# cheneeheng/2s-AGCN

Hardware: AMD Instinct MI355X
Metric: skeleton-clips/sec fwd+bwd, NTU (N,3,300,25,2) (higher is better)
Workload: dtype f32; 1 GPU; AGCN joint-stream NTU-xview shape, full training step (fwd, CE, bwd, grad all-reduce, clip 1.0, SGD nesterov); per_gpu_batch=64, global_batch=64, input=(N,3,300,25,2), parallelism=dp1, bn=per-replica

## Files before the change

2s-agcn_amd/csrc/bn.hip:

```cpp
#include "agcn_common.h"

namespace {

constexpr int RG = 64;

__global__ void __launch_bounds__(256)
colsum_stage1_kernel(const float* __restrict__ X, int nslots, int W, int per_group, double* __restrict__ partial) {
  __shared__ double red[4][64];
  const int col = blockIdx.x * 64 + (threadIdx.x & 63), sub = threadIdx.x >> 6;
  const int g = blockIdx.y;
  const int s_end = min(nslots, (g + 1) * per_group);
  double acc = 0.0;
  if (col < W)
    for (int s = g * per_group + sub; s < s_end; s += 4) acc += (double)X[(long)s * W + col];
  red[sub][threadIdx.x & 63] = acc;
  __syncthreads();
  if (sub == 0 && col < W)
    partial[(long)g * W + col] = red[0][threadIdx.x] + red[1][threadIdx.x] + red[2][threadIdx.x] + red[3][threadIdx.x];
}

__global__ void colsum_stage2_kernel(const double* __restrict__ partial, int W, float* __restrict__ out) {
  const int col = blockIdx.x * blockDim.x + threadIdx.x;
  if (col >= W) return;
  double s = 0.0;
  for (int g = 0; g < RG; ++g) s += partial[(long)g * W + col];
  out[col] = (float)s;
}

__global__ void bn_stats_finalize_kernel(const double* __restrict__ partial, int C, double count,
                                         const float* __restrict__ gamma, const float* __restrict__ beta,
                                         float* __restrict__ rmean, float* __restrict__ rvar, float momentum,
                                         float eps, float* __restrict__ mean_out, float* __restrict__ invstd_out,
                                         float* __restrict__ scale_out, float* __restrict__ shift_out) {
  const int c = blockIdx.x * blockDim.x + threadIdx.x;
  if (c >= C) return;
  double s = 0.0, ss = 0.0;
  for (int g = 0; g < RG; ++g) {
    s += partial[((long)g * 2 + 0) * C + c];
    ss += partial[((long)g * 2 + 1) * C + c];
  }
  const double mean = s / count;
  double var = ss / count - mean * mean;
  if (var < 0.0) var = 0.0;
  const float invstd = (float)(1.0 / sqrt(var + (double)eps));
  mean_out[c] = (float)mean;
  invstd_out[c] = invstd;
  const float sc = gamma[c] * invstd;
  scale_out[c] = sc;
  shift_out[c] = beta[c] - (float)mean * sc;
  if (rmean) {
    const double unb = count > 1.0 ? var * count / (count - 1.0) : var;
    rmean[c] = (1.f - momentum) * rmean[c] + momentum * (float)mean;
    rvar[c] = (1.f - momentum) * rvar[c] + momentum * (float)unb;
  }
}

__global__ void bn_eval_coeff_kernel(const float* __restrict__ gamma, const float* __restrict__ beta,
                                     const float* __restrict__ rmean, const float* __restrict__ rvar, float eps, int C,
                                     float* __restrict__ scale_out, float* __restrict__ shift_out) {
  const int c = blockIdx.x * blockDim.x + threadIdx.x;
  if (c >= C) return;
  const float sc = gamma[c] / sqrtf(rvar[c] + eps);
  scale_out[c] = sc;
  shift_out[c] = beta[c] - rmean[c] * sc;
}

template <int RES, bool RELU>
__global__ void __launch_bounds__(256)
bn_act_fwd_kernel(const float4* __restrict__ y1, const float* __restrict__ scale1, const float* __restrict__ shift1,
                  const float4* __restrict__ r, const float* __restrict__ scale2, const float* __restrict__ shift2,
                  float4* __restrict__ out, unsigned* __restrict__ bits, unsigned total4, unsigned P, unsigned C,
                  unsigned* __restrict__ amax) {
  unsigned tmax = 0;
  for (unsigned i0 = blockIdx.x * blockDim.x; i0 < total4; i0 += gridDim.x * blockDim.x) {
    const unsigned i = i0 + threadIdx.x;
    const bool valid = i < total4;
    const unsigned ic = valid ? i : 0u;
    const unsigned e0 = ic * 4u;
    const unsigned row = e0 / P;
    const unsigned rem = e0 - row * P;
    const unsigned c0 = row % C;
    const unsigned c1 = (c0 + 1 == C) ? 0u : c0 + 1;
    const float4 a = y1[ic];
    float4 b = make_float4(0.f, 0.f, 0.f, 0.f);
    if (RES != 0) b = r[ic];
    float av[4] = {a.x, a.y, a.z, a.w};
    float bv[4] = {b.x, b.y, b.z, b.w};
    float ov[4];
#pragma unroll
    for (int k = 0; k < 4; ++k) {
      const unsigned c = (rem + k < P) ? c0 : c1;
      float v = scale1[c] * av[k] + shift1[c];
      if (RES == 1) v += bv[k];
      if (RES == 2) v += scale2[c] * bv[k] + shift2[c];
      ov[k] = RELU ? fmaxf(v, 0.f) : v;
    }
    if (valid) out[i] = make_float4(ov[0], ov[1], ov[2], ov[3]);
    if (amax && valid) {
#pragma unroll
      for (int k = 0; k < 4; ++k) tmax = max(tmax, __float_as_uint(ov[k]) & 0x7fffffffu);
    }
    if (bits) {
      unsigned nib = valid ? ((ov[0] > 0.f) | ((ov[1] > 0.f) << 1) | ((ov[2] > 0.f) << 2) | ((ov[3] > 0.f) << 3)) : 0u;
      unsigned w = nib << (4u * (threadIdx.x & 7u));
      w |= __shfl_xor(w, 1);
      w |= __shfl_xor(w, 2);
      w |= __shfl_xor(w, 4);
      if ((threadIdx.x & 7u) == 0u && valid) bits[e0 >> 5] = w;
    }
  }
  if (amax) {
#pragma unroll
    for (int k = 32; k >= 1; k >>= 1) tmax = max(tmax, (unsigned)__shfl_xor((int)tmax, k));
    __shared__ unsigned wmax[4];
    if ((threadIdx.x & 63u) == 0u) wmax[threadIdx.x >> 6] = tmax;
    __syncthreads();
    if (threadIdx.x == 0) {
      const unsigned m = max(max(wmax[0], wmax[1]), max(wmax[2], wmax[3]));
      if (m) atomicMax(amax, m);
    }
  }
}

template <bool HAS2>
__global__ void __launch_bounds__(256)
bn_bwd_reduce_kernel(const float* __restrict__ dout, const float* __restrict__ mask, int mask_bits,
                     const float* __restrict__ y1, const float* __restrict__ y2, float* __restrict__ part, int P) {
  __shared__ float red[3][4];
  const long row = blockIdx.x;
  const float* d = dout + row * P;
  const float* mk = (mask && !mask_bits) ? mask + row * P : nullptr;
  const unsigned* mb = (mask && mask_bits) ? reinterpret_cast<const unsigned*>(mask) : nullptr;
  const long e_row = row * P;
  const float* a = y1 + row * P;
  const float* b = HAS2 ? y2 + row * P : nullptr;
  float s0 = 0.f, s1 = 0.f, s2 = 0.f;
  typedef float4 float4_u __attribute__((aligned(4)));
  const int P4 = P >> 2;
  for (int q4 = threadIdx.x; q4 < P4; q4 += 256) {
    const float4 d4 = reinterpret_cast<const float4_u*>(d)[q4];
    const float4 a4 = reinterpret_cast<const float4_u*>(a)[q4];
    float dv[4] = {d4.x, d4.y, d4.z, d4.w};
    const float av[4] = {a4.x, a4.y, a4.z, a4.w};
    if (mk) {
      const float4 m4 = reinterpret_cast<const float4_u*>(mk)[q4];
      const float mv[4] = {m4.x, m4.y, m4.z, m4.w};
#pragma unroll
      for (int k = 0; k < 4; ++k) dv[k] = (mv[k] > 0.f) ? dv[k] : 0.f;
    }
    if (mb) {
      const long e = e_row + 4L * q4;
      const int sh = (int)(e & 31);
      unsigned nib = mb[e >> 5] >> sh;
      if (sh > 28) nib |= mb[(e >> 5) + 1] << (32 - sh);
#pragma unroll
      for (int k = 0; k < 4; ++k) dv[k] = ((nib >> k) & 1u) ? dv[k] : 0.f;
    }
    float bv[4] = {0.f, 0.f, 0.f, 0.f};
    if (HAS2) {
      const float4 b4 = reinterpret_cast<const float4_u*>(b)[q4];
      bv[0] = b4.x; bv[1] = b4.y; bv[2] = b4.z; bv[3] = b4.w;
    }
#pragma unroll
    for (int k = 0; k < 4; ++k) {
      s0 += dv[k];
      s1 += dv[k] * av[k];
      if (HAS2) s2 += dv[k] * bv[k];
    }
  }
  for (int q = 4 * P4 + threadIdx.x; q < P; q += 256) {
    float dz = d[q];
    if (mk) dz = (mk[q] > 0.f) ? dz : 0.f;
    if (mb) {
      const long e = e_row + q;
      dz = ((mb[e >> 5] >> (e & 31)) & 1u) ? dz : 0.f;
    }
    s0 += dz;
    s1 += dz * a[q];
    if (HAS2) s2 += dz * b[q];
  }
  s0 = half_sum(s0); s1 = half_sum(s1); s2 = half_sum(s2);
  s0 += __shfl_xor(s0, 32); s1 += __shfl_xor(s1, 32); s2 += __shfl_xor(s2, 32);
  const int wave = threadIdx.x >> 6;
  if ((threadIdx.x & 63) == 0) { red[0][wave] = s0; red[1][wave] = s1; red[2][wave] = s2; }
  __syncthreads();
  if (threadIdx.x < 3) {
    const int k = threadIdx.x;
    part[row * 3 + k] = red[k][0] + red[k][1] + red[k][2] + red[k][3];
  }
}

__global__ void bn_bwd_finalize_kernel(const float* __restrict__ part, int N, int C, double count, float pscale,
                                       const float* __restrict__ gamma1, const float* __restrict__ mean1,
                                       const float* __restrict__ invstd1, const float* __restrict__ gamma2,
                                       const float* __restrict__ mean2, const float* __restrict__ invstd2,
                                       float* __restrict__ coef, float* __restrict__ dgamma1,
                                       float* __restrict__ dbeta1, float* __restrict__ dgamma2,
                                       float* __restrict__ dbeta2) {
  const int c = blockIdx.x * blockDim.x + threadIdx.x;
  if (c >= C) return;
  double s0 = 0.0, s1 = 0.0, s2 = 0.0;
#pragma unroll 8
  for (int n = 0; n < N; ++n) {
    const float* p = part + ((long)n * C + c) * 3;
    s0 += (double)p[0]; s1 += (double)p[1]; s2 += (double)p[2];
  }
  {
    const double is = invstd1[c], mu = mean1[c], g = gamma1[c];
    const double sxh = is * (s1 - mu * s0);
    const double k = g * is;
    coef[0 * C + c] = (float)k;
    coef[1 * C + c] = (float)(-k * is * sxh / count);
    coef[2 * C + c] = (float)(-k * s0 / count + k * is * mu * sxh / count);
    dgamma1[c] = (float)sxh * pscale;
    dbeta1[c] = (float)s0 * pscale;
  }
  if (gamma2) {
    const double is = invstd2[c], mu = mean2[c], g = gamma2[c];
    const double sxh = is * (s2 - mu * s0);
    const double k = g * is;
    coef[3 * C + c] = (float)k;
    coef[4 * C + c] = (float)(-k * is * sxh / count);
    coef[5 * C + c] = (float)(-k * s0 / count + k * is * mu * sxh / count);
    dgamma2[c] = (float)sxh * pscale;
    dbeta2[c] = (float)s0 * pscale;
  }
}

template <bool HAS2>
__global__ void __launch_bounds__(256)
bn_bwd_apply_kernel(const float4* __restrict__ dout, const float4* __restrict__ mask, int mask_bits,
                    const float4* __restrict__ y1,
                    const float4* __restrict__ y2, const float* __restrict__ coef, float4* __restrict__ dy1,
                    float4* __restrict__ dy2, unsigned total4, unsigned P, unsigned C, unsigned* __restrict__ amax1) {
  unsigned tmax = 0;
  for (unsigned i = blockIdx.x * blockDim.x + threadIdx.x; i < total4; i += gridDim.x * blockDim.x) {
    const unsigned e0 = i * 4u;
    const unsigned row = e0 / P;
    const unsigned rem = e0 - row * P;
    const unsigned c0 = row % C;
    const unsigned c1 = (c0 + 1 == C) ? 0u : c0 + 1;
    const float4 d4 = dout[i];
    const float4 a4 = y1[i];
    float dv[4] = {d4.x, d4.y, d4.z, d4.w};
    float av[4] = {a4.x, a4.y, a4.z, a4.w};
    if (mask && !mask_bits) {
      const float4 m4 = mask[i];
      const float mv[4] = {m4.x, m4.y, m4.z, m4.w};
#pragma unroll
      for (int k = 0; k < 4; ++k) dv[k] = (mv[k] > 0.f) ? dv[k] : 0.f;
    } else if (mask) {
      const unsigned nib = reinterpret_cast<const unsigned*>(mask)[e0 >> 5] >> (e0 & 31u);
#pragma unroll
      for (int k = 0; k < 4; ++k) dv[k] = ((nib >> k) & 1u) ? dv[k] : 0.f;
    }
    float bv[4] = {0.f, 0.f, 0.f, 0.f};
    if (HAS2) {
      const float4 b4 = y2[i];
      bv[0] = b4.x; bv[1] = b4.y; bv[2] = b4.z; bv[3] = b4.w;
    }
    float o1[4], o2[4];
#pragma unroll
    for (int k = 0; k < 4; ++k) {
      const unsigned c = (rem + k < P) ? c0 : c1;
      o1[k] = coef[0 * C + c] * dv[k] + coef[1 * C + c] * av[k] + coef[2 * C + c];
      if (HAS2) o2[k] = coef[3 * C + c] * dv[k] + coef[4 * C + c] * bv[k] + coef[5 * C + c];
    }
    dy1[i] = make_float4(o1[0], o1[1], o1[2], o1[3]);
    if (HAS2) dy2[i] = make_float4(o2[0], o2[1], o2[2], o2[3]);
    if (amax1) {
#pragma unroll
      for (int k = 0; k < 4; ++k) tmax = max(tmax, __float_as_uint(o1[k]) & 0x7fffffffu);
    }
  }
  if (amax1) {
#pragma unroll
    for (int k = 32; k >= 1; k >>= 1) tmax = max(tmax, (unsigned)__shfl_xor((int)tmax, k));
    __shared__ unsigned wmax[4];
    if ((threadIdx.x & 63u) == 0u) wmax[threadIdx.x >> 6] = tmax;
    __syncthreads();
    if (threadIdx.x == 0) {
      const unsigned m = max(max(wmax[0], wmax[1]), max(wmax[2], wmax[3]));
      if (m) atomicMax(amax1, m);
    }
  }
}

inline unsigned ew_grid(unsigned total4) {
  unsigned g = (total4 + 255u) / 256u;
  return g > 4096u ? 4096u : (g ? g : 1u);
}

}

extern "C" {

size_t agcn_colsum_scratch_bytes(int W) { return sizeof(double) * (size_t)RG * (size_t)W; }

int agcn_colsum(const float* X, int nslots, int W, void* scratch, float* out, void* stream) {
  if (!X || !scratch || !out || nslots <= 0 || W <= 0) return AGCN_ERR_ARG;
  hipStream_t s = (hipStream_t)stream;
  const int per_group = (nslots + RG - 1) / RG;
  hipLaunchKernelGGL(colsum_stage1_kernel, dim3((W + 63) / 64, RG), dim3(256), 0, s, X, nslots, W, per_group,
                     (double*)scratch);
  int rc = agcn_check_launch();
  if (rc) return rc;
  hipLaunchKernelGGL(colsum_stage2_kernel, dim3((W + 255) / 256), dim3(256), 0, s, (const double*)scratch, W, out);
  return agcn_check_launch();
}

int agcn_bn_stats_finalize(const float* part, int nslots, int C, double count, const float* gamma, const float* beta,
                           float* running_mean, float* running_var, float momentum, float eps, void* scratch,
                           float* mean, float* invstd, float* scale, float* shift, void* stream) {
  if (!part || !gamma || !beta || !scratch || !mean || !invstd || !scale || !shift || C <= 0 || nslots <= 0)
    return AGCN_ERR_ARG;
  hipStream_t s = (hipStream_t)stream;
  const int W = 2 * C;
  const int per_group = (nslots + RG - 1) / RG;
  hipLaunchKernelGGL(colsum_stage1_kernel, dim3((W + 63) / 64, RG), dim3(256), 0, s, part, nslots, W, per_group,
                     (double*)scratch);
  int rc = agcn_check_launch();
  if (rc) return rc;
  hipLaunchKernelGGL(bn_stats_finalize_kernel, dim3((C + 63) / 64), dim3(64), 0, s, (const double*)scratch, C, count,
                     gamma, beta, running_mean, running_var, momentum, eps, mean, invstd, scale, shift);
  return agcn_check_launch();
}

int agcn_bn_eval_coeff(const float* gamma, const float* beta, const float* running_mean, const float* running_var,
                       float eps, int C, float* scale, float* shift, void* stream) {
  if (!gamma || !beta || !running_mean || !running_var || !scale || !shift || C <= 0) return AGCN_ERR_ARG;
  hipLaunchKernelGGL(bn_eval_coeff_kernel, dim3((C + 63) / 64), dim3(64), 0, (hipStream_t)stream, gamma, beta,
                     running_mean, running_var, eps, C, scale, shift);
  return agcn_check_launch();
}

int agcn_bn_act_fwd(const float* y1, const float* scale1, const float* shift1, const float* r, const float* scale2,
                    const float* shift2, float* out, unsigned* sign_bits, int N, int C, int P, int res_mode, int relu,
                    void* stream) {
  return agcn_bn_act_fwd_ex(y1, scale1, shift1, r, scale2, shift2, out, sign_bits, nullptr, N, C, P, res_mode, relu, stream);
}

int agcn_bn_act_fwd_ex(const float* y1, const float* scale1, const float* shift1, const float* r, const float* scale2,
                       const float* shift2, float* out, unsigned* sign_bits, float* absmax_out, int N, int C, int P,
                       int res_mode, int relu, void* stream) {
  if (!y1 || !scale1 || !shift1 || !out || N <= 0 || C <= 0 || P <= 0) return AGCN_ERR_ARG;
  if (absmax_out && hipMemsetAsync(absmax_out, 0, 4, (hipStream_t)stream) != hipSuccess) return AGCN_ERR_ARG;
  const long total = (long)N * C * P;
  if (total % 4 != 0 || total > 0xffffffffL) return AGCN_ERR_UNSUPPORTED;
  if (res_mode != 0 && !r) return AGCN_ERR_ARG;
  if (res_mode == 2 && (!scale2 || !shift2)) return AGCN_ERR_ARG;
  const unsigned t4 = (unsigned)(total / 4);
  hipStream_t s = (hipStream_t)stream;
  const dim3 g(ew_grid(t4)), b(256);
#define LAUNCH_ACT(R, A)                                                                                       \
  hipLaunchKernelGGL((bn_act_fwd_kernel<R, A>), g, b, 0, s, (const float4*)y1, scale1, shift1, (const float4*)r, \
                     scale2, shift2, (float4*)out, sign_bits, t4, (unsigned)P, (unsigned)C, (unsigned*)absmax_out)
  if (relu) {
    if (res_mode == 0) LAUNCH_ACT(0, true); else if (res_mode == 1) LAUNCH_ACT(1, true); else LAUNCH_ACT(2, true);
  } else {
    if (res_mode == 0) LAUNCH_ACT(0, false); else if (res_mode == 1) LAUNCH_ACT(1, false); else LAUNCH_ACT(2, false);
  }
#undef LAUNCH_ACT
  return agcn_check_launch();
}

int agcn_bn_bwd_reduce(const float* dout, const void* mask, int mask_bits, const float* y1, const float* y2, float* part,
                       int N, int C, int P, void* stream) {
  if (!dout || !y1 || !part || N <= 0 || C <= 0 || P <= 0) return AGCN_ERR_ARG;
  hipStream_t s = (hipStream_t)stream;
  if (y2) hipLaunchKernelGGL(bn_bwd_reduce_kernel<true>, dim3(N * C), dim3(256), 0, s, dout, (const float*)mask,
                             mask_bits, y1, y2, part, P);
  else hipLaunchKernelGGL(bn_bwd_reduce_kernel<false>, dim3(N * C), dim3(256), 0, s, dout, (const float*)mask,
                          mask_bits, y1, y2, part, P);
  return agcn_check_launch();
}

int agcn_bn_bwd_apply(const float* part, int nrows, double count, float param_grad_scale, const float* dout,
                      const void* mask, int mask_bits, const float* y1, const float* gamma1, const float* mean1, const float* invstd1,
                      const float* y2, const float* gamma2, const float* mean2, const float* invstd2, float* coef,
                      float* dy1, float* dgamma1, float* dbeta1, float* dy2, float* dgamma2, float* dbeta2, int N, int C,
                      int P, void* stream) {
  return agcn_bn_bwd_apply_ex(part, nrows, count, param_grad_scale, dout, mask, mask_bits, y1, gamma1, mean1, invstd1, y2,
                              gamma2, mean2, invstd2, coef, dy1, dgamma1, dbeta1, dy2, dgamma2, dbeta2, nullptr, N, C, P,
                              stream);
}

int agcn_bn_bwd_apply_ex(const float* part, int nrows, double count, float param_grad_scale, const float* dout,
                         const void* mask, int mask_bits, const float* y1, const float* gamma1, const float* mean1,
                         const float* invstd1, const float* y2, const float* gamma2, const float* mean2,
                         const float* invstd2, float* coef, float* dy1, float* dgamma1, float* dbeta1, float* dy2,
                         float* dgamma2, float* dbeta2, float* absmax1_out, int N, int C, int P, void* stream) {
  if (absmax1_out && hipMemsetAsync(absmax1_out, 0, 4, (hipStream_t)stream) != hipSuccess) return AGCN_ERR_ARG;
  if (!part || !dout || !y1 || !gamma1 || !mean1 || !invstd1 || !coef || !dy1 || !dgamma1 || !dbeta1 || nrows <= 0)
    return AGCN_ERR_ARG;
  if (y2 && (!gamma2 || !mean2 || !invstd2 || !dy2 || !dgamma2 || !dbeta2)) return AGCN_ERR_ARG;
  const long total = (long)N * C * P;
  if (total % 4 != 0 || total > 0xffffffffL) return AGCN_ERR_UNSUPPORTED;
  hipStream_t s = (hipStream_t)stream;
  hipLaunchKernelGGL(bn_bwd_finalize_kernel, dim3((C + 63) / 64), dim3(64), 0, s, part, nrows, C, count,
                     param_grad_scale, gamma1, mean1, invstd1, y2 ? gamma2 : nullptr, mean2, invstd2, coef, dgamma1,
                     dbeta1, dgamma2, dbeta2);
  int rc = agcn_check_launch();
  if (rc) return rc;
  const unsigned t4 = (unsigned)(total / 4);
  const dim3 g(ew_grid(t4)), b(256);
  if (y2)
    hipLaunchKernelGGL(bn_bwd_apply_kernel<true>, g, b, 0, s, (const float4*)dout, (const float4*)mask, mask_bits,
                       (const float4*)y1, (const float4*)y2, (const float*)coef, (float4*)dy1, (float4*)dy2, t4,
                       (unsigned)P, (unsigned)C, (unsigned*)absmax1_out);
  else
    hipLaunchKernelGGL(bn_bwd_apply_kernel<false>, g, b, 0, s, (const float4*)dout, (const float4*)mask, mask_bits,
                       (const float4*)y1, (const float4*)y2, (const float*)coef, (float4*)dy1, (float4*)dy2, t4,
                       (unsigned)P, (unsigned)C, (unsigned*)absmax1_out);
  return agcn_check_launch();
}

int agcn_bn_bwd(const float* dout, const void* mask, int mask_bits, const float* y1, const float* gamma1,
                const float* mean1, const float* invstd1, const float* y2, const float* gamma2, const float* mean2,
                const float* invstd2, float* part, float* coef, float* dy1, float* dgamma1, float* dbeta1, float* dy2,
                float* dgamma2, float* dbeta2, int N, int C, int P, void* stream) {
  int rc = agcn_bn_bwd_reduce(dout, mask, mask_bits, y1, y2, part, N, C, P, stream);
  if (rc) return rc;
  return agcn_bn_bwd_apply(part, N, (double)N * (double)P, 1.0f, dout, mask, mask_bits, y1, gamma1, mean1, invstd1, y2, gamma2,
                           mean2, invstd2, coef, dy1, dgamma1, dbeta1, dy2, dgamma2, dbeta2, N, C, P, stream);
}

const char* agcn_arch(void) { return "gfx950"; }
int agcn_version(void) { return 100; }

}
```

2s-agcn_amd/lib.py:

```python
import ctypes
import os
import re

import torch

_HERE = os.path.dirname(os.path.abspath(__file__))
LIB_PATH = os.path.join(_HERE, "libagcn_hip.so")
HEADER_PATH = os.path.join(os.path.dirname(_HERE), "include", "agcn_hip.h")

_RETURNS = {"int": ctypes.c_int, "size_t": ctypes.c_size_t, "const char*": ctypes.c_char_p}
_SCALARS = {"int": ctypes.c_int, "long": ctypes.c_long, "size_t": ctypes.c_size_t, "float": ctypes.c_float,
            "double": ctypes.c_double}
_FP32, _FP64, _INT32 = ("fp32", (torch.float32,)), ("float64", (torch.float64,)), ("int32", (torch.int32,))
_BITS32, _ANY = ("int32", (torch.int32, torch.uint32)), ("", None)
_POINTERS = {"float*": _FP32, "const float*": _FP32, "double*": _FP64, "const double*": _FP64,
             "int*": _INT32, "const int*": _INT32, "unsigned*": _BITS32, "const unsigned*": _BITS32,
             "const long long*": ("int64", (torch.int64,)), "const unsigned char*": ("uint8", (torch.uint8,)),
             "void*": _ANY, "const void*": _ANY}
_TYPE_WORDS = {"const", "void", "char", "int", "long", "unsigned", "signed", "short", "float", "double", "size_t"}


def _c_type(tokens):
    return " ".join(tokens).replace(" *", "*")


def parse_header(text):
    text = re.sub(r"/\*.*?\*/|//[^\n]*", " ", text, flags=re.S)
    codes = {m.group(1): int(m.group(2))
             for m in re.finditer(r"^[ \t]*#[ \t]*define[ \t]+(AGCN_\w+)[ \t]+\(?(-?\d+)\)?[ \t]*$", text, flags=re.M)}
    text = re.sub(r"^[ \t]*#.*$", " ", text, flags=re.M)
    text = re.sub(r'extern\s+"C"\s*\{', " ", text)
    decls = {}
    for chunk in text.split(";"):
        decl = " ".join(chunk.split())
        if decl in ("", "}"):
            continue
        m = re.fullmatch(r"([\w\s*]+?)\b(\w+) ?\(([^()]*)\)", decl)
        if m is None:
            raise RuntimeError(f"agcn_amd: cannot read the declaration `{decl}` of the C ABI header")
        ret, name = _c_type(m.group(1).replace("*", " * ").split()), m.group(2)
        if ret not in _RETURNS:
            raise RuntimeError(f"agcn_amd: return type `{ret}` outside the binding's set in `{decl}`")
        params = []
        for p in ([] if m.group(3).strip() in ("", "void") else m.group(3).split(",")):
            tokens = p.replace("*", " * ").split()
            if len(tokens) < 2 or tokens[-1] == "*" or tokens[-1] in _TYPE_WORDS:
                raise RuntimeError(f"agcn_amd: parameter `{p.strip()}` has no name in `{decl}`")
            ctype = _c_type(tokens[:-1])
            if ctype not in _SCALARS and ctype not in _POINTERS:
                raise RuntimeError(f"agcn_amd: parameter type `{ctype}` outside the binding's set in `{decl}`")
            params.append((ctype, tokens[-1]))
        decls[name] = (ret, params)
    return decls, codes


def _read_header():
    try:
        with open(HEADER_PATH) as f:
            return f.read()
    except OSError as e:
        raise RuntimeError(f"agcn_amd: the C ABI header {HEADER_PATH} is missing ({e}); the binding is derived from "
                           f"it") from e


def _pointer_converter(ctype, where):
    kind, dtypes = _POINTERS[ctype]
    want = f"{where}: expected a contiguous {kind + ' ' if kind else ''}GPU tensor"

    def convert(t):
        if t is None or type(t) is int:
            return t
        if not (t.is_cuda and t.is_contiguous() and (dtypes is None or t.dtype in dtypes)):
            raise RuntimeError(f"agcn_amd: {want}, got {t.dtype} {tuple(t.shape)} on {t.device} "
                               f"contiguous={t.is_contiguous()}")
        return t.data_ptr()
    return convert


def _host_ints_converter(where):
    def convert(values):
        if values is None:
            return None
        if torch.is_tensor(values):
            if values.is_cuda or values.dtype.is_floating_point or values.dtype == torch.bool:
                raise RuntimeError(f"agcn_amd: {where}: expected a host sequence of ints, got {values.dtype} on "
                                   f"{values.device}")
            values = values.tolist()
        values = list(values)
        if any(isinstance(v, bool) or int(v) != v for v in values):
            raise RuntimeError(f"agcn_amd: {where}: expected a host sequence of ints, got {values!r}")
        return (ctypes.c_int * len(values))(*[int(v) for v in values])
    return convert


def _converter(ctype, pname, name):
    if pname.startswith("host_"):
        assert ctype == "const int*", f"{name}({pname}): host arrays are `const int*`"
        return _host_ints_converter(f"{name}({pname})")
    return _pointer_converter(ctype, f"{name}({pname})")


DECLARATIONS, _CODES = parse_header(_read_header())
ERR_ARG, ERR_WORKSPACE, ERR_UNSUPPORTED = (_CODES[k] for k in ("AGCN_ERR_ARG", "AGCN_ERR_WORKSPACE",
                                                                "AGCN_ERR_UNSUPPORTED"))
SIGNATURES = {name: (_RETURNS[ret], [_SCALARS.get(t, ctypes.c_void_p) for t, _ in params])
              for name, (ret, params) in DECLARATIONS.items()}
_CONVERTERS = {}
for _name, (_ret, _params) in DECLARATIONS.items():
    if any(t in _POINTERS for t, _ in _params):
        assert _ret == "int" and _params[-1] == ("void*", "stream"), f"{_name}: not `int {_name}(..., void* stream)`"
        _CONVERTERS[_name] = tuple(_converter(t, p, _name) if t in _POINTERS else None for t, p in _params[:-1])

_lib = None


def load():
    global _lib
    if _lib is not None:
        return _lib
    if not os.path.exists(LIB_PATH):
        raise RuntimeError(
            f"agcn_amd: HIP extension {LIB_PATH} not found -- run `python -c 'import __graft_entry__ as g; "
            f"g.build()'` (hipcc --offload-arch=gfx950).  There is no CPU fallback for the hot path.")
    lib = ctypes.CDLL(LIB_PATH)
    for name, (res, args) in SIGNATURES.items():
        fn = getattr(lib, name)
        fn.restype = res
        fn.argtypes = args
    _lib = lib
    return lib


ptr = _pointer_converter("const float*", "ptr")
ptr.__doc__ = "Device pointer of a tensor (None -> NULL).  The tensor must be contiguous fp32 on a GPU."
ptr_bits = _pointer_converter("const int*", "ptr_bits")
ptr_bits.__doc__ = "Device pointer of an int32 sign-bit-mask tensor (None -> NULL)."


def stream():
    return torch.cuda.current_stream().cuda_stream


def check(rc, what):
    if rc != 0:
        raise RuntimeError(f"agcn_amd: {what} failed with code {rc}")


def status(name, *args):
    convert = _CONVERTERS.get(name)
    if convert is None:
        raise RuntimeError(f"agcn_amd: {name} is not a stream entry point of include/agcn_hip.h")
    if len(args) != len(convert):
        raise RuntimeError(f"agcn_amd: {name} takes {len(convert)} arguments in front of the stream, got {len(args)}")
    return getattr(_lib or load(), name)(*[a if c is None else c(a) for c, a in zip(convert, args)], stream())


def call(name, *args):
    check(status(name, *args), name)
```

2s-agcn_amd/model/agcn.py:

```python
import math

import numpy as np
import torch
import torch.nn as nn

from .. import ops


def import_class(name):
    import importlib
    module_name, _, cls = name.rpartition('.')
    return getattr(importlib.import_module(module_name), cls)


def conv_branch_init(conv, branches):
    out_c, in_c, k = conv.weight.size(0), conv.weight.size(1), conv.weight.size(2)
    nn.init.normal_(conv.weight, 0, math.sqrt(2.0 / (out_c * in_c * k * branches)))
    nn.init.constant_(conv.bias, 0)


def conv_init(conv):
    nn.init.kaiming_normal_(conv.weight, mode='fan_out')
    nn.init.constant_(conv.bias, 0)


def bn_init(bn, scale):
    nn.init.constant_(bn.weight, scale)
    nn.init.constant_(bn.bias, 0)


def _require_gpu(x, who):
    if not x.is_cuda:
        raise RuntimeError(f"agcn_amd.{who}: input is on {x.device}; the hot path exists only as gfx950 HIP kernels "
                           f"(no CPU fallback). Move the model and data to a GPU.")
    if x.dtype != torch.float32:
        raise RuntimeError(f"agcn_amd.{who}: expected float32 input, got {x.dtype}")


def _bn_args(bn):
    return bn.weight, bn.bias, bn.running_mean, bn.running_var


def _bn_tick(bn, training):
    if training and bn.num_batches_tracked is not None:
        bn.num_batches_tracked.add_(1)


def _conv_bn_args(conv, bn):
    return (conv.weight, conv.bias) + _bn_args(bn)


def gcn_params(g, ab, A, PA, alpha=None):
    return dict(conv_d=[(c.weight, c.bias) for c in g.conv_d],
                ab=None if ab is None else [(a.weight, a.bias, b.weight, b.bias) for a, b in zip(ab.conv_a, ab.conv_b)],
                A=A, PA=PA, alpha=alpha, gbn=_bn_args(g.bn),
                down=_conv_bn_args(*g.down) if isinstance(g.down, nn.Sequential) else None)


def unit_params(unit, p, attn=None):
    t, r = unit.tcn1, unit.residual
    p.update(tw=t.conv.weight, tb=t.conv.bias, tbn=_bn_args(t.bn), res_mode=unit.res_mode,
             res=_conv_bn_args(r.conv, r.bn) if unit.res_mode == 2 else None, stride=unit.stride, pad=t.pad, attn=attn)
    return p


def data_bn_forward(bn, x):
    N, C, T, V, M = x.size()
    if ops.data_bn_supported(bn):
        y = ops.DataBNFunction.apply(x, bn.weight, bn.bias, bn.running_mean, bn.running_var, bn.training,
                                     ops.sync_of(bn))
        _bn_tick(bn, bn.training)
        return y
    x = x.permute(0, 4, 3, 1, 2).contiguous().view(N, M * V * C, T)
    x = bn(x)
    return x.view(N, M, V, C, T).permute(0, 1, 3, 4, 2).contiguous().view(N * M, C, T, V)


class unit_tcn(nn.Module):
    def __init__(self, in_channels, out_channels, kernel_size=9, stride=1):
        super().__init__()
        if not 1 <= kernel_size <= 9:
            raise NotImplementedError(f"agcn_amd.unit_tcn: kernel_size {kernel_size} is outside 1..9, the temporal "
                                      f"kernel sizes the HIP convolution kernels are built for")
        pad = int((kernel_size - 1) / 2)
        self.conv = nn.Conv2d(in_channels, out_channels, kernel_size=(kernel_size, 1), padding=(pad, 0),
                              stride=(stride, 1))
        self.bn = nn.BatchNorm2d(out_channels)
        self.relu = nn.ReLU()
        self.stride, self.pad = stride, pad
        conv_init(self.conv)
        bn_init(self.bn, 1)

    def forward(self, x):
        _require_gpu(x, 'unit_tcn')
        y = ops.UnitTCNFunction.apply(x, self.conv.weight, self.conv.bias, *_bn_args(self.bn), self.stride,
                                      self.training, ops.sync_of(self.bn), self.pad)
        _bn_tick(self.bn, self.training)
        return y


class unit_gcn(nn.Module):
    def __init__(self, in_channels, out_channels, A, coff_embedding=4, num_subset=3):
        super().__init__()
        if num_subset != 3:
            raise ValueError("agcn_amd.unit_gcn: num_subset must be 3")
        inter_channels = out_channels // coff_embedding
        self.inter_c = inter_channels
        self.in_channels, self.out_channels = in_channels, out_channels
        A = np.asarray(A, dtype=np.float32)
        self.PA = nn.Parameter(torch.full(A.shape, 1e-6, dtype=torch.float32))
        self.register_buffer('A', torch.from_numpy(A.copy()), persistent=False)
        self.num_subset = num_subset
        self.conv_a = nn.ModuleList()
        self.conv_b = nn.ModuleList()
        self.conv_d = nn.ModuleList()
        for _ in range(num_subset):
            self.conv_a.append(nn.Conv2d(in_channels, inter_channels, 1))
            self.conv_b.append(nn.Conv2d(in_channels, inter_channels, 1))
            self.conv_d.append(nn.Conv2d(in_channels, out_channels, 1))
        if in_channels != out_channels:
            self.down = nn.Sequential(nn.Conv2d(in_channels, out_channels, 1), nn.BatchNorm2d(out_channels))
        else:
            self.down = lambda x: x
        self.bn = nn.BatchNorm2d(out_channels)
        self.soft = nn.Softmax(-2)
        self.relu = nn.ReLU()
        for m in self.modules():
            if isinstance(m, nn.Conv2d):
                conv_init(m)
            elif isinstance(m, nn.BatchNorm2d):
                bn_init(m, 1)
        bn_init(self.bn, 1e-6)
        for i in range(num_subset):
            conv_branch_init(self.conv_d[i], num_subset)

    def params(self):
        return gcn_params(self, self, self.A, self.PA)

    def tick(self):
        _bn_tick(self.bn, self.training)
        if isinstance(self.down, nn.Sequential):
            _bn_tick(self.down[1], self.training)

    def forward(self, x):
        _require_gpu(x, 'unit_gcn')
        y = ops.UnitGCNFunction.apply(x, *ops.pack_gcn(self.params()), self.training, None, ops.sync_of(self.bn))
        self.tick()
        return y


class TCN_GCN_unit(nn.Module):
    def __init__(self, in_channels, out_channels, A, stride=1, residual=True):
        super().__init__()
        self.gcn1 = unit_gcn(in_channels, out_channels, A)
        self.tcn1 = unit_tcn(out_channels, out_channels, stride=stride)
        self.relu = nn.ReLU()
        self.stride = stride
        if not residual:
            self.residual = lambda x: 0
            self.res_mode = 0
        elif (in_channels == out_channels) and (stride == 1):
            self.residual = lambda x: x
            self.res_mode = 1
        else:
            self.residual = unit_tcn(in_channels, out_channels, kernel_size=1, stride=stride)
            self.res_mode = 2

    def train(self, mode=True):
        self.__dict__.pop('_infer_cache', None)
        return super().train(mode)

    def forward(self, x):
        _require_gpu(x, 'TCN_GCN_unit')
        t = self.tcn1
        p = unit_params(self, self.gcn1.params())
        if not self.training and not torch.is_grad_enabled() and ops.infer_fold_enabled():
            y = ops.unit_infer(x, p, cache=self.__dict__.setdefault('_infer_cache', {}))
            if y is not None:
                return y
        y = ops.TCNGCNUnitFunction.apply(x, *ops.pack_gcn(p), *ops.pack_tcn(p), self.training, ops.sync_of(t.bn))
        self.gcn1.tick()
        _bn_tick(t.bn, self.training)
        if self.res_mode == 2:
            _bn_tick(self.residual.bn, self.training)
        return y


class Model(nn.Module):
    def __init__(self, num_class=60, num_point=25, num_person=2, graph=None, graph_args=dict(), in_channels=3):
        super().__init__()
        if graph is None:
            raise ValueError()
        Graph = import_class(graph) if isinstance(graph, str) else graph
        self.graph = Graph(**graph_args)
        A = self.graph.A
        self.data_bn = nn.BatchNorm1d(num_person * in_channels * num_point)
        self.l1 = TCN_GCN_unit(3, 64, A, residual=False)
        self.l2 = TCN_GCN_unit(64, 64, A)
        self.l3 = TCN_GCN_unit(64, 64, A)
        self.l4 = TCN_GCN_unit(64, 64, A)
        self.l5 = TCN_GCN_unit(64, 128, A, stride=2)
        self.l6 = TCN_GCN_unit(128, 128, A)
        self.l7 = TCN_GCN_unit(128, 128, A)
        self.l8 = TCN_GCN_unit(128, 256, A, stride=2)
        self.l9 = TCN_GCN_unit(256, 256, A)
        self.l10 = TCN_GCN_unit(256, 256, A)
        self.fc = nn.Linear(256, num_class)
        nn.init.normal_(self.fc.weight, 0, math.sqrt(2. / num_class))
        bn_init(self.data_bn, 1)

    def forward(self, x):
        N, C, T, V, M = x.size()
        _require_gpu(x, 'Model')
        x = data_bn_forward(self.data_bn, x)
        for k in range(1, 11):
            x = getattr(self, f'l{k}')(x)
        return ops.PoolFCFunction.apply(x, self.fc.weight, self.fc.bias, M)
```

2s-agcn_amd/ops.py:

```python
import collections
import math
import os
import weakref

import numpy as np
import torch

from . import lib as _lib

BN_EPS = 1e-5
BN_MOMENTUM = 0.1


def _L():
    return _lib.load()


def _empty(shape, like):
    return torch.empty(shape, dtype=torch.float32, device=like.device)


def _ws(nbytes, like):
    return torch.empty((int(nbytes) + 3) // 4, dtype=torch.float32, device=like.device)

# ... 129 lines not shown
    _lib.call("agcn_adjacency_fwd", tp, A, PA, alpha, spart, P, adj, N, Ci, T, V)
    return P, adj


def adjacency_fused_supported(C, Ci, T, V):
    return bool(_L().agcn_adjacency_fused_supported(int(C), int(Ci), int(T), int(V)))


def adjacency_recompute():
    return os.environ.get('AGCN_ADJ_RECOMPUTE', '0') == '1'


def adjacency_fused_fwd(x, wab, bab, A, PA, alpha=None, keep_tp=False, x_amax_out=None, x_amax=None):
    N, C, T, V = x.shape
    Ci = wab.shape[0] // 6
    tp = _empty((N, 6 * Ci, T, V), x) if keep_tp else None
    nt = _L().agcn_scores_num_tiles(V, T)
    spart = _empty((N, 3, nt, V, V), x)
    P = _empty((N, 3, V, V), x)
    adj = _empty((N, 3, V, V), x)
    nb = _L().agcn_adjacency_fused_workspace(C, Ci)
    ws = _ws(nb, x)
    _lib.call("agcn_adjacency_fused_fwd_ex", x, wab.reshape(6 * Ci, C), bab, A, PA, alpha, tp, spart, P, adj,
              x_amax_out, x_amax, ws, nb, N, C, Ci, T, V)
    return (P, adj, tp) if keep_tp else (P, adj)


def first_layer_enabled():
    return os.environ.get('AGCN_FIRST_LAYER', '1') != '0'


def gcn_first_fwd(x, adj, wcat, bias, wdown, bdown, want_stats=False):
    N, C, T, V = x.shape
    Cout = wcat.shape[0]
    ypre, dpre = _empty((N, Cout, T, V), x), _empty((N, Cout, T, V), x)
    st = st2 = None
    if want_stats:
        nt = _L().agcn_gcn_first_tiles(T, V)
        st, st2 = _empty((N * nt, 2, Cout), x), _empty((N * nt, 2, Cout), x)
    wdown2 = wdown.reshape(Cout, C).contiguous()
    _lib.call("agcn_gcn_first_fwd", x, adj, wcat, bias, wdown2, bdown, ypre, st, dpre, st2, N, C, Cout, T, V)
    return ypre, st, dpre, st2


def aggregate_project_fwd(x, adj, wcat, bias, want_stats=False, x_amax=None):
    N, C, T, V = x.shape
    Cout = wcat.shape[0]
    y = _empty((N, Cout, T, V), x)
    stats = None
    if want_stats:
        stats = _empty((_L().agcn_gcn_stats_slots(N, C, Cout, T, V), 2, Cout), x)
    ws, nb = _gcn_ws(C, Cout, T, V, x)
    _lib.call("agcn_gcn_aggregate_project_fwd_ex", x, adj, wcat, bias, y, stats, ws, nb, N, C, Cout, T, V, x_amax)
    return y, stats


def aggregate_project_bwd_data(dy, adj, wcat, x_shape, out=None, accumulate=False, add1=None, mask1=None,
                               add2=None, mask2=None, dtp=None, wab=None, dy_amax=None, dtp_amax=None):
    N, C, T, V = x_shape
    Cout = wcat.shape[0]
    dx = out if out is not None else _empty(x_shape, dy)
    ws, nb = _gcn_ws(C, Cout, T, V, dy)
    kinds = {m.dtype for m in (mask1, mask2) if m is not None}
    if len(kinds) > 1:
        raise RuntimeError("agcn_amd: mask1 and mask2 must be of one kind (fp32 tensors or int32 sign bit masks)")
    mbits = int(torch.int32 in kinds)
    mp = _lib.ptr_bits if mbits else _lib.ptr
    K2, w2 = 0, None
    if dtp is not None:
        K2 = dtp.shape[1]
        w2 = wab.reshape(K2, C)
    else:
        dtp_amax = None
    _lib.call("agcn_gcn_aggregate_project_bwd_data_ex", dy, adj, wcat, dtp, w2, K2, dx, int(accumulate), add1,
              mp(mask1), add2, mp(mask2), mbits, ws, nb, N, C, Cout, T, V, dy_amax, dtp_amax)
    return dx


def fused_bwd_data_supported(C, Cout, V):
    return bool(_L().agcn_gcn_bwd_data_fused_supported(int(C), int(Cout), int(V)))


def project_bwd_weight(dy, x, adj, Cout, dy_amax=None, x_amax=None):
    N, C, T, V = x.shape
    nbytes = _L().agcn_gcn_project_bwd_weight_workspace(N, C, Cout, T, V)
    ws = torch.empty((nbytes + 3) // 4, dtype=torch.float32, device=x.device)
    dw = _empty((Cout, 3 * C), x)
    _lib.call("agcn_gcn_project_bwd_weight_ex", dy, x, adj, dw, ws, nbytes, N, C, Cout, T, V, dy_amax, x_amax)
    return dw


def adjacency_bwd(dy, wcat, x, tp, P, alpha=None, wab=None, bab=None, dy_amax=None, x_amax=None):
    N, C, T, V = x.shape
    Cout = wcat.shape[0]
    Ci = (tp.shape[1] if tp is not None else wab.shape[0]) // 6
    nslots = _L().agcn_dadj_num_slots(C, V, T)
    dpart = _empty((N, 3, nslots, V, V), x)
    ws, nb = _gcn_ws(C, Cout, T, V, x)
    _lib.call("agcn_gcn_dadj_ex", dy, wcat, x, dpart, ws, nb, N, C, Cout, T, V, dy_amax, x_amax)
    dadj = _empty((N, 3, V, V), x)
    dS = _empty((N, 3, V, V), x)
    dPA = _empty((3, V, V), x)
    dal_part = _empty((N * 3,), x) if alpha is not None else None
    _lib.call("agcn_adjacency_bwd_softmax", dpart, P, alpha, dadj, dS, dPA, dal_part, N, Ci, T, V, nslots)
    nt = _L().agcn_scores_num_tiles(V, T)
    dtp = _empty((N, 6 * Ci, T, V), x)
    dbpart = _empty((N * nt, 6 * Ci), x)
    dbab = _empty((6 * Ci,), x)
    scratch = _scratch(6 * Ci, x)
    dtp_amax = None
    if tp is None:
        nb = _L().agcn_adjacency_fused_workspace(C, Ci)
        ws = _ws(nb, x)
        _lib.call("agcn_adjacency_fused_bwd_scores", x, wab.reshape(6 * Ci, C), bab, dS, dtp, dbpart, scratch, dbab, ws,
                  nb, N, C, Ci, T, V)
    else:
        dtp_amax = _empty((1,), x) if fused_amax_enabled() else None
        _lib.call("agcn_adjacency_bwd_scores_ex", tp, dS, dtp, dbpart, scratch, dbab, dtp_amax, N, Ci, T, V)
    dalpha = dal_part.sum() if dal_part is not None else None
    return dPA, dtp, dbab, dalpha, dadj, dtp_amax


def stc_row_reduce(y, g=None, wv=None, wt=None, want_t=False, want_v=False, scale_t=1.0, scale_v=1.0):
    N, C, T, V = y.shape
    out_t = _empty((N, C, T), y) if want_t else None
    out_v = _empty((N, C, V), y) if want_v else None
    per_row = int(wt is not None and wt.dim() == 3)
    _lib.call("agcn_stc_row_reduce", y, g, wv, wt, per_row, out_t, out_v, float(scale_t), float(scale_v), N, C, T, V)
    return out_t, out_v


def linear_fwd(x, w, b, act=0):
    N, K = x.shape
    O = w.shape[0]
    out = _empty((N, O), x)
    _lib.call("agcn_linear_fwd", x, w, b, out, N, K, O, int(act))
    return out


def linear_bwd(dout, out, x, w, act=0, need_din=True):
    N, K = x.shape
    O = w.shape[0]
    dpre = _empty((N, O), x)
    din = _empty((N, K), x) if need_din else None
    dw, db = _empty((O, K), x), _empty((O,), x)
    _lib.call("agcn_linear_bwd", dout, out, x, w, dpre, din, dw, db, N, K, O, int(act))
    return din, dw, db


def gate_conv_fwd(x, w, b):
    N, C, L = x.shape
    Ks = w.shape[-1]
    a = _empty((N, L), x)
    _lib.call("agcn_gate_conv_fwd", x, w.reshape(C, Ks), b, a, N, C, L, Ks)
    return a


def gate_conv_bwd(da, a, x, w):
    N, C, L = x.shape
    Ks = w.shape[-1]
    dpre = _empty((N, L), x)
    dx, dw, db = _empty((N, C, L), x), _empty((1, C, Ks), x), _empty((1,), x)
    _lib.call("agcn_gate_conv_bwd", da, a, x, w.reshape(C, Ks), dpre, dx, dw, db, N, C, L, Ks)
    return dx, dw, db


class DataBNFunction(torch.autograd.Function):

    @staticmethod
    def forward(ctx, x, w, b, rm, rv, training, sync=None):
        x = x.contiguous()
        N, C, T, V, M = x.shape
        CH = C * V * M
        if training:
            part = _empty((N, 2, CH), x)
            _lib.call("agcn_data_bn_stats", x, part, N, C, T, V, M)
            (st,), gcount = _bn_coeffs(True, [part], N * T, [(w, b, rm, rv)], sync, N)
        else:
            (st,), gcount = _bn_coeffs(False, [None], N * T, [(w, b, rm, rv)], None, N)
        out = _empty((N * M, C, T, V), x)
        _lib.call("agcn_data_bn_apply", x, st.scale, st.shift, out, N, C, T, V, M)
        ctx.st, ctx.sync, ctx.gcount, ctx.training = st, sync, gcount, training
        ctx.save_for_backward(x, w)
        return out

    @staticmethod
    def backward(ctx, dy):
        x, w = ctx.saved_tensors
        st, sync = ctx.st, ctx.sync
        dy = dy.contiguous()
        N, C, T, V, M = x.shape
        CH = C * V * M
        ng = ctx.needs_input_grad
        sums = None
        if ctx.training or ng[1] or ng[2]:
            part = _empty((N, 2, CH), x)
            _lib.call("agcn_data_bn_bwd_reduce", dy, x, st.mean, st.invstd, part, N, C, T, V, M)
            sums = _colsum(part, N, 2 * CH)
        scale = 1.0
        if ctx.training and sync is not None:
            sums = _allreduce_sum(sums, sync)
            scale = 1.0 / sync.world
        dx = dgamma = dbeta = None
        if ng[0]:
            dx = torch.empty_like(x)
            corr = sums if ctx.training else torch.zeros(2 * CH, dtype=torch.float32, device=x.device)
            _lib.call("agcn_data_bn_bwd_apply", dy, x, w, st.mean, st.invstd, corr, float(ctx.gcount), dx, N, C, T, V,
                      M)
        if sums is not None:
            dbeta, dgamma = sums[:CH], sums[CH:]
            if scale != 1.0:
                dbeta, dgamma = dbeta * scale, dgamma * scale
        return dx, dgamma, dbeta, None, None, None, None


def data_bn_supported(bn):
    return type(bn) in (torch.nn.BatchNorm1d, torch.nn.SyncBatchNorm)


class PoolFCFunction(torch.autograd.Function):

    @staticmethod
    def forward(ctx, x, w, b, M):
        x = x.contiguous()
        NM, C, T, V = x.shape
        N = NM // M
        rowmean, pooled = _empty((NM, C), x), _empty((N, C), x)
        _lib.call("agcn_pool_fwd", x, rowmean, pooled, N, M, C, T * V)
        logits = linear_fwd(pooled, w, b, 0)
        ctx.save_for_backward(pooled, logits, w)
        ctx.shape, ctx.M = (NM, C, T, V), M
        return logits

    @staticmethod
    def backward(ctx, dlogits):
        pooled, logits, w = ctx.saved_tensors
        NM, C, T, V = ctx.shape
        M = ctx.M
        dpooled, dw, db = linear_bwd(dlogits.contiguous(), logits, pooled, w, 0, need_din=True)
        dx = None
        if ctx.needs_input_grad[0]:
            dx = _empty((NM, C, T, V), pooled)
            _lib.call("agcn_pool_bwd", dpooled, dx, NM // M, M, C, T * V)
        return dx, dw, db, None


class STCAttentionFunction(torch.autograd.Function):

    @staticmethod
    def _gates(m_s, mv1, sa_w, sa_b, ta_w, ta_b, f1w, f1b, f2w, f2b, a_s=None):
        if a_s is None:
            a_s = gate_conv_fwd(m_s, sa_w, sa_b)
        if mv1 is None:
            return a_s, None, None, None, None
        a_t = gate_conv_fwd(mv1, ta_w, ta_b)
        m_c = (mv1 * a_t.unsqueeze(1)).mean(-1)
        h = linear_fwd(m_c, f1w, f1b, 1)
        a_c = linear_fwd(h, f2w, f2b, 2)
        return a_s, a_t, a_c, m_c, h

    @staticmethod
    def forward(ctx, y, sa_w, sa_b, ta_w, ta_b, f1w, f1b, f2w, f2b):
        y = y.contiguous()
        N, C, T, V = y.shape
        par = (sa_w, sa_b, ta_w, ta_b, f1w, f1b, f2w, f2b)
        _, m_s = stc_row_reduce(y, want_v=True, scale_v=1.0 / T)
        a_s = STCAttentionFunction._gates(m_s, None, *par)[0]
        mv1, _ = stc_row_reduce(y, wv=a_s, want_t=True, scale_t=1.0 / V)
        _, a_t, a_c, m_c, h = STCAttentionFunction._gates(m_s, mv1, *par, a_s=a_s)
        out = torch.empty_like(y)
        o_amax = _empty((1,), y) if fused_amax_enabled() else None
        INFER_STATS['stc_apply'] += 1
        _lib.call("agcn_stc_apply_ex", y, a_s, a_t, a_c, out, o_amax, N, C, T, V)
        _note_out_amax(out, o_amax)
        ctx.save_for_backward(y, m_s, mv1, a_s, a_t, a_c, m_c, h, *par)
        return out

    @staticmethod
    def backward(ctx, dout):
        y, m_s, mv1, a_s, a_t, a_c, m_c, h, *par = ctx.saved_tensors
        sa_w, sa_b, ta_w, ta_b, f1w, f1b, f2w, f2b = par
        dout = dout.contiguous()
        N, C, T, V = y.shape
        P1, P2 = stc_row_reduce(y, g=dout, wv=a_s, wt=a_t, want_t=True, want_v=True)
        da_c = (P1 * a_t.unsqueeze(1)).sum(-1).contiguous()
        da_t = (P1 * a_c.unsqueeze(-1)).sum(1)
        da_s = (P2 * a_c.unsqueeze(-1)).sum(1)
        dh, df2w, df2b = linear_bwd(da_c, a_c, h, f2w, 2)
        dm_c, df1w, df1b = linear_bwd(dh, h, m_c, f1w, 1)
        da_t = (da_t + (dm_c.unsqueeze(-1) * mv1).sum(1) / T).contiguous()
        dmv1 = dm_c.unsqueeze(-1) * a_t.unsqueeze(1) / T
        dmv1_t, dta_w, dta_b = gate_conv_bwd(da_t, a_t, mv1, ta_w)
        dmv1 = ((dmv1 + dmv1_t) / V).contiguous()
        _, R = stc_row_reduce(y, wt=dmv1, want_v=True)
        da_s = (da_s + R.sum(1)).contiguous()
        dm_s, dsa_w, dsa_b = gate_conv_bwd(da_s, a_s, m_s, sa_w)
        dms = (dm_s / T).contiguous()
        dy = torch.empty_like(y)
        _lib.call("agcn_stc_bwd_apply", dout, a_s, a_t, a_c, dmv1, dms, dy, N, C, T, V)
        return dy, dsa_w, dsa_b, dta_w, dta_b, df1w, df1b, df2w, df2b


class BNState:
    __slots__ = ("mean", "invstd", "scale", "shift", "S", "eval")

    def __init__(self):
        self.S = 1
        self.eval = False


class SyncBN:
    __slots__ = ("world", "group")

    def __init__(self, world, group=None):
        self.world, self.group = int(world), group


def sync_of(bn_module):
    import torch.distributed as dist
    if isinstance(bn_module, torch.nn.SyncBatchNorm) and dist.is_available() and dist.is_initialized():
        world = dist.get_world_size(bn_module.process_group)
        if world > 1:
            return SyncBN(world, bn_module.process_group)
    return None


def _colsum(slab, nslots, width):
    out = _empty((width,), slab)
    scratch = _scratch(width, slab)
    _lib.call("agcn_colsum", slab, int(nslots), int(width), scratch, out)
    return out


COLLECTIVES = {'bn': 0, 'grad': 0}


def _allreduce_sum(t, sync):
    import torch.distributed as dist
    COLLECTIVES['bn'] += 1
    dist.all_reduce(t, op=dist.ReduceOp.SUM, group=sync.group)
    return t


def sync_stats(stats_parts, count, sync):
    sums = [_colsum(sp, sp.shape[0], sp.shape[1] * sp.shape[2]) for sp in stats_parts]
    buf = torch.cat(sums) if len(sums) > 1 else sums[0]
    _allreduce_sum(buf, sync)
    out, o = [], 0
    for sp in stats_parts:
        w = sp.shape[1] * sp.shape[2]
        out.append(buf[o:o + w].view(1, 2, sp.shape[2]))
        o += w
    return out


def bn_train_coeffs(stats_part, count, gamma, beta, running_mean, running_var, momentum=BN_MOMENTUM, eps=BN_EPS):
    C = gamma.numel()
    st = BNState()
    st.mean, st.invstd = _empty((C,), gamma), _empty((C,), gamma)
    st.scale, st.shift = _empty((C,), gamma), _empty((C,), gamma)
    nslots = stats_part.shape[0]
    scratch = _scratch(2 * C, gamma)
    _lib.call("agcn_bn_stats_finalize", stats_part, nslots, C, float(count), gamma, beta, running_mean, running_var,
              float(momentum), float(eps), scratch, st.mean, st.invstd, st.scale, st.shift)
    return st


def bn_eval_coeffs(gamma, beta, running_mean, running_var, eps=BN_EPS):
    C = gamma.numel()
    st = BNState()
    st.eval = True
    st.scale, st.shift = _empty((C,), gamma), _empty((C,), gamma)
    st.mean, st.invstd = _empty((C,), gamma), _empty((C,), gamma)
    _lib.call("agcn_bn_eval_coeff_ex", gamma, beta, running_mean, running_var, float(eps), C, st.scale, st.shift,
              st.mean, st.invstd)
    return st


def bn_act_fwd(y1, st1, r=None, st2=None, relu=True, want_bits=False, amax_out=None):
    N, C, T, V = y1.shape
    if st1.S > 1:
        N, C = N // st1.S, C * st1.S
    out = torch.empty_like(y1)
    bits = torch.empty((y1.numel() + 31) // 32, dtype=torch.int32, device=y1.device) if want_bits else None
    mode = 0 if r is None else (1 if st2 is None else 2)
    _lib.call("agcn_bn_act_fwd_ex", y1, st1.scale, st1.shift, r, st2.scale if st2 else None, st2.shift if st2 else None,
              out, bits, amax_out, N, C, T * V, mode, int(relu))
    return (out, bits) if want_bits else out


EVAL_BWD_STATS = {'sums': 0, 'nosums': 0}


def _mask_arg(mask):
    mbits = int(mask is not None and mask.dtype == torch.int32)
    return (_lib.ptr_bits(mask) if mbits else _lib.ptr(mask)), mbits


def bn_bwd_eval(dout, mask, y1, st1, y2=None, st2=None, want_sums=True, amax_out=None):
    N, C, T, V = dout.shape
    two = st2 is not None
    dy1 = torch.empty_like(dout)
    dy2 = torch.empty_like(dout) if two else None
    part = _empty((N * C * 3,), dout) if want_sums else None
    mptr, mbits = _mask_arg(mask)
    EVAL_BWD_STATS['sums' if want_sums else 'nosums'] += 1
    _lib.call("agcn_bn_bwd_eval", dout, mptr, mbits, y1 if want_sums else None, st1.scale,
              y2 if (want_sums and two) else None, st2.scale if two else None, int(want_sums), part, dy1, dy2, amax_out,
              N, C, T * V)
    if not want_sums:
        return dy1, None, None, None, dy2, None, None, None
    dg1, db1, dc1 = _empty((C,), dout), _empty((C,), dout), _empty((C,), dout)
    dg2 = db2 = dc2 = None
    if two:
        dg2, db2, dc2 = _empty((C,), dout), _empty((C,), dout), _empty((C,), dout)
    _lib.call("agcn_bn_bwd_eval_finalize", part, N, C, st1.scale, st1.mean, st1.invstd, st2.scale if two else None,
              st2.mean if two else None, st2.invstd if two else None, dg1, db1, dc1, dg2, db2, dc2)
    return dy1, dg1, db1, dc1, dy2, dg2, db2, dc2


def _bn_bwd_two_stage(grad, ins, outs, part, coef, amax_out, N, C, TV, sync, gcount):
    dout, mptr, mbits = grad
    _lib.call("agcn_bn_bwd_reduce", dout, mptr, mbits, ins[0], ins[4], part, N, C, TV)
    sums, nslots, total, scale = part, N, float(N) * float(TV), 1.0
    if sync is not None:
        sums, nslots, scale = _allreduce_sum(_colsum(part, N, 3 * C), sync), 1, 1.0 / sync.world
        total = float(gcount) if gcount is not None else total * sync.world
    _lib.call("agcn_bn_bwd_apply_ex", sums, nslots, total, scale, dout, mptr, mbits, *ins, coef, *outs, amax_out, N, C,
              TV)


def bn_bwd(dout, mask, y1, gamma1, st1, y2=None, gamma2=None, st2=None, sync=None, gcount=None, amax_out=None,
           want_sums=True, bias_out=None):
    if st1.eval:
        dy1, dg1, db1, dc1, dy2, dg2, db2, dc2 = bn_bwd_eval(dout, mask, y1, st1, y2, st2 if y2 is not None else None,
                                                             want_sums, amax_out)
        if bias_out is not None:
            bias_out[:] = [dc1, dc2]
        return dy1, dg1, db1, dy2, dg2, db2
    N, C, T, V = y1.shape
    S = st1.S
    if S > 1:
        N, C = N // S, C * S
        gamma1 = gamma1.repeat(S)
        gamma2 = gamma2.repeat(S) if gamma2 is not None else None
    part = _empty((N * C * 3,), y1)
    coef = _empty((6 * C,), y1)
    dy1 = torch.empty_like(y1)
    dg1, db1 = _empty((C,), y1), _empty((C,), y1)
    dy2 = dg2 = db2 = None
    if y2 is not None:
        dy2 = torch.empty_like(y2)
        dg2, db2 = _empty((C,), y1), _empty((C,), y1)
    grad = (dout, *_mask_arg(mask))
    ins = (y1, gamma1, st1.mean, st1.invstd, y2, gamma2, st2.mean if st2 else None, st2.invstd if st2 else None)
    outs = (dy1, dg1, db1, dy2, dg2, db2)
    if sync is None and amax_out is None:
        _lib.call("agcn_bn_bwd", *grad, *ins, part, coef, *outs, N, C, T * V)
    else:
        _bn_bwd_two_stage(grad, ins, outs, part, coef, amax_out, N, C, T * V, sync, gcount)
    if S > 1:
        dg1, db1 = dg1.view(S, -1).sum(0), db1.view(S, -1).sum(0)
        if dg2 is not None:
            dg2, db2 = dg2.view(S, -1).sum(0), db2.view(S, -1).sum(0)
    return dy1, dg1, db1, dy2, dg2, db2



class _GCNState:
    __slots__ = ('x', 'tp', 'P', 'adj', 'ypre', 'dpre', 'bits', 'bn1', 'bn2', 'sync', 'count', 'x_amax', 'g_amax',
                 'wab', 'bab', 'wd', 'gamma1', 'wdown', 'gamma2', 'alpha')

    def __init__(self, x, tp, P, adj, ypre, dpre, bits, bn1, bn2, sync, count, x_amax, g_amax, wab, bab, wd, gamma1,
                 wdown, gamma2, alpha):
        self.x, self.tp, self.P, self.adj, self.ypre, self.dpre, self.bits = x, tp, P, adj, ypre, dpre, bits
        self.bn1, self.bn2, self.sync, self.count, self.x_amax, self.g_amax = bn1, bn2, sync, count, x_amax, g_amax
        self.wab, self.bab, self.wd, self.gamma1, self.wdown, self.gamma2 = wab, bab, wd, gamma1, wdown, gamma2
        self.alpha = alpha


class _TCNState:
    __slots__ = ('g', 'zpre', 'rpre', 'out', 'bits', 'bn1', 'bn2', 'sync', 'count', 'g_amax', 'resx', 'w', 'gamma1',
                 'wres', 'gamma2', 'stride', 'relu', 'pad')

    def __init__(self, g, zpre, rpre, out, bits, bn1, bn2, sync, count, g_amax, resx, w, gamma1, wres, gamma2, stride,
                 relu, pad):
        self.g, self.zpre, self.rpre, self.out, self.bits, self.bn1, self.bn2 = g, zpre, rpre, out, bits, bn1, bn2
        self.sync, self.count, self.g_amax, self.resx, self.w, self.gamma1 = sync, count, g_amax, resx, w, gamma1
        self.wres, self.gamma2, self.stride, self.relu, self.pad = wres, gamma2, stride, relu, pad


def _bn_coeffs(training, stats, count, bns, sync=None, nsamples=None):
    S = bns[0][2].numel() // bns[0][0].numel()
    if not training:
        out = []
        for w, b, rm, rv in bns:
            C = w.numel()
            out.append(bn_eval_coeffs(w, b, rm[:C].contiguous(), rv[:C].contiguous()))
        return out, count
    if S > 1:
        if nsamples is None or nsamples % S:
            raise RuntimeError(f"agcn_amd: GhostBatchNorm with {S} splits needs a batch (x persons) divisible by {S}")
        stats = [_ghost_regroup(sp, S, nsamples) for sp in stats]
        bns = [(w.repeat(S), b.repeat(S), rm, rv) for w, b, rm, rv in bns]
        count = count // S
    if sync is not None:
        stats = sync_stats(stats, count, sync)
        count = count * sync.world
    note_params_changed()
    res = [bn_train_coeffs(sp, count, *bn) for sp, bn in zip(stats, bns)]
    for st in res:
        st.S = S
    return res, count


def _ghost_regroup(stats_part, S, nsamples):
    slots, two, C = stats_part.shape
    nt = slots // nsamples
    return stats_part.view(nsamples // S, S, nt, two, C).permute(0, 2, 3, 1, 4).reshape(nsamples // S * nt, two, S * C)


def _adjacency(x, wab, bab, A, PA, alpha, *, keep_tp, x_amax, want_amax):
    N, C, T, V = x.shape
    if wab is None:
        return None, A.unsqueeze(0).expand(N, 3, V, V).contiguous(), None, x_amax
    if not adjacency_fused_supported(C, wab.shape[0] // 6, T, V):
        tp, _ = conv_fwd(x, wab, bab)
        P, adj = adjacency_fwd(tp, A, PA, alpha)
        return P, adj, tp, x_amax
    amax_here = _empty((1,), x) if want_amax and x_amax is None and fused_amax_enabled() else None
    if keep_tp and not adjacency_recompute():
        P, adj, tp = adjacency_fused_fwd(x, wab, bab, A, PA, alpha, keep_tp=True, x_amax_out=amax_here, x_amax=x_amax)
    else:
        tp = None
        P, adj = adjacency_fused_fwd(x, wab, bab, A, PA, alpha, x_amax_out=amax_here, x_amax=x_amax)
    return P, adj, tp, x_amax if amax_here is None else amax_here


def gcn_forward(x, A, PA, wab, bab, wd, bd, bn, down, training, alpha=None, sync=None, need_bwd=True):
    N, C, T, V = x.shape
    count = N * T * V
    first = down is not None and first_layer_enabled() and bool(_L().agcn_gcn_first_supported(C, wd.shape[0], V))
    x_amax = None if first else _take_out_amax(x)
    P, adj, tp, x_amax = _adjacency(x, wab, bab, A, PA, alpha, keep_tp=need_bwd, x_amax=x_amax, want_amax=not first)
    if first:
        ypre, st, dpre, st2 = gcn_first_fwd(x, adj, wd, bd, down[0], down[1], want_stats=training)
    else:
        ypre, st = aggregate_project_fwd(x, adj, wd, bd, want_stats=training, x_amax=x_amax)
        dpre, st2 = conv_fwd(x, down[0], down[1], want_stats=training) if down is not None else (None, None)
    if down is not None:
        (bn1, bn2), gcount = _bn_coeffs(training, [st, st2], count, [bn, down[2:]], sync, N)
        r = dpre
    else:
        (bn1,), gcount = _bn_coeffs(training, [st], count, [bn], sync, N)
        bn2, r = None, x
    g_amax = _empty((1,), x) if fused_amax_enabled() else None
    out, bits = bn_act_fwd(ypre, bn1, r, bn2, relu=True, want_bits=True, amax_out=g_amax)
    wdown, gamma2 = (down[0], down[2]) if down is not None else (None, None)
    return out, _GCNState(x, tp, P, adj, ypre, dpre, bits, bn1, bn2, sync, gcount, x_amax, g_amax, wab, bab, wd, bn[0],
                          wdown, gamma2, alpha)


def _bias_grad(slot, k, n, like, needed=True):
    if slot and slot[k] is not None:
        return slot[k]
    if slot:
        return None
    return torch.zeros(n, dtype=torch.float32, device=like.device) if needed else None


def gcn_backward(s, dout, extra_add=None, extra_mask=None, want_sums=True):
    x, tp, adj, ypre, dpre, wab, wd, wdown = s.x, s.tp, s.adj, s.ypre, s.dpre, s.wab, s.wd, s.wdown
    Cout = wd.shape[0]
    dy_amax = _empty((1,), dout) if fused_amax_enabled() else None
    dbias = []
    dypre, dg1, db1, ddpre, dg2, db2 = bn_bwd(dout, s.bits, ypre, s.gamma1, s.bn1, dpre, s.gamma2, s.bn2, sync=s.sync,
                                              gcount=s.count, amax_out=dy_amax, want_sums=want_sums, bias_out=dbias)
    x_amax = s.x_amax
    dwd = _side_run(lambda: project_bwd_weight(dypre, x, adj, Cout, dy_amax, x_amax), (dypre, x, adj, dy_amax, x_amax))
    dPA = dwab = dbab = dalpha = dtp = dtp_amax = None
    if wab is not None:
        dPA, dtp, dbab, dalpha, _, dtp_amax = adjacency_bwd(dypre, wd, x, tp, s.P, s.alpha, wab, s.bab,
                                                            dy_amax=dy_amax, x_amax=x_amax)
        dwab = _side_run(lambda: conv_bwd_weight(dtp, x, wab.shape, 1, dtp_amax, x_amax), (dtp, x, dtp_amax, x_amax))
    fuse = dtp is not None and fused_bwd_data_supported(x.shape[1], Cout, x.shape[3])
    ftp = dict(dtp=dtp, wab=wab, dtp_amax=dtp_amax) if fuse else {}
    if dpre is None:
        dx = aggregate_project_bwd_data(dypre, adj, wd, x.shape, add1=dout, mask1=s.bits, add2=extra_add,
                                        mask2=extra_mask, dy_amax=dy_amax, **ftp)
    else:
        dx = aggregate_project_bwd_data(dypre, adj, wd, x.shape, add1=extra_add, mask1=extra_mask, dy_amax=dy_amax,
                                        **ftp)
    if dtp is not None and not fuse:
        conv_bwd_data(dtp, wab, x.shape, out=dx, accumulate=True)
    dwdown = None
    if dpre is not None:
        dwdown = _side_run(lambda: conv_bwd_weight(ddpre, x, wdown.shape), (ddpre, x))
        conv_bwd_data(ddpre, wdown, x.shape, out=dx, accumulate=True)
    _side_join()
    dbd = _bias_grad(dbias, 0, Cout, dout)
    dbdown = _bias_grad(dbias, 1, Cout, dout, dpre is not None)
    return dx, dPA, dwab, dbab, dwd, dbd, dg1, db1, dwdown, dbdown, dg2, db2, dalpha


def tcn_forward(g, w, b, bn, stride, res_x, res, relu, training, sync=None, pad=None, g_amax=None):
    N, C, T, V = g.shape
    if res is not None:
        To = conv_out_frames(T, w.shape[2], stride, pad)
        Tr = res_x.shape[2] if isinstance(res, str) else conv_out_frames(res_x.shape[2], 1, stride, 0)
        if Tr != To:
            raise RuntimeError(f"agcn_amd: the residual has {Tr} frames but the temporal convolution ({w.shape[2]} taps, "
                               f"stride {stride}, padding {(w.shape[2] - 1) // 2 if pad is None else pad}) gives {To} "
                               f"for {T} input frames; they must agree (the reference fails here too)")
    zpre, st = conv_fwd(g, w, b, stride, want_stats=training, x_amax=g_amax, pad=pad)
    To = zpre.shape[2]
    count = N * To * V
    rpre = bn2 = wres = gamma2 = None
    if res is None or isinstance(res, str):
        (bn1,), gcount = _bn_coeffs(training, [st], count, [bn], sync, N)
        r = None if res is None else res_x
    else:
        r, st2 = conv_fwd(res_x, res[0], res[1], stride, want_stats=training)
        (bn1, bn2), gcount = _bn_coeffs(training, [st, st2], count, [bn, res[2:]], sync, N)
        rpre, wres, gamma2 = r, res[0], res[2]
    o_amax = _empty((1,), g) if fused_amax_enabled() else None
    out, bits = bn_act_fwd(zpre, bn1, r, bn2, relu=relu, want_bits=True, amax_out=o_amax)
    _note_out_amax(out, o_amax)
    return out, _TCNState(g, zpre, rpre, out, bits, bn1, bn2, sync, gcount, g_amax, res_x, w, bn[0], wres, gamma2,
                          stride, relu, pad)


def tcn_backward(s, dout, join=True, want_sums=True):
    w, wres, g, stride, pad, g_amax = s.w, s.wres, s.g, s.stride, s.pad, s.g_amax
    mask = s.bits if s.relu else None
    dz_amax = _empty((1,), dout) if fused_amax_enabled() else None
    dbias = []
    dzpre, dg1, db1, drpre, dg2, db2 = bn_bwd(dout, mask, s.zpre, s.gamma1, s.bn1, s.rpre, s.gamma2, s.bn2, sync=s.sync,
                                              gcount=s.count, amax_out=dz_amax, want_sums=want_sums, bias_out=dbias)
    dw = _side_run(lambda: conv_bwd_weight(dzpre, g, w.shape, stride, dz_amax, g_amax, pad=pad),
                   (dzpre, g, dz_amax, g_amax))
    dg = conv_bwd_data(dzpre, w, g.shape, stride, dy_amax=dz_amax, pad=pad)
    dwres = None
    if drpre is not None:
        resx = s.resx
        dwres = _side_run(lambda: conv_bwd_weight(drpre, resx, wres.shape, stride), (drpre, resx))
    if join:
        _side_join()
    Cout = w.shape[0]
    return (dg, dw, _bias_grad(dbias, 0, Cout, dout), dg1, db1,
            drpre, dwres, _bias_grad(dbias, 1, Cout, dout, drpre is not None), dg2, db2)


ERR_UNSUPPORTED = _lib.ERR_UNSUPPORTED


def _launched(name, *args):
    rc = _lib.status(name, *args)
    if rc != ERR_UNSUPPORTED:
        _lib.check(rc, name)
    return rc != ERR_UNSUPPORTED

_PARAM_EPOCH = [0]


def note_params_changed():
    _PARAM_EPOCH[0] += 1


def infer_fold_enabled():
    return os.environ.get('AGCN_INFER_FOLD', '1') != '0'


INFER_STATS = {'aagcn_unit_fused': 0, 'tconv_infer': 0, 'stc_apply': 0}


def _fold(bn):
    w, b, rm, rv = bn
    C = w.numel()
    s = w / torch.sqrt(rv[:C] + BN_EPS)
    return s, b - rm[:C] * s


def _fold_conv(w, b, bn):
    s, sh = _fold(bn)
    return (w * s[:, None, None, None]).contiguous(), (b * s + sh).contiguous()


def gcn_unit_infer(x, adj, wcat, bias, res=None, x2=None, w2=None, relu=True):
    N, C, T, V = x.shape
    Cout = wcat.shape[0]
    K2 = 0 if x2 is None else x2.shape[1]
    nbytes = _L().agcn_gcn_unit_infer_workspace(C, Cout, K2, T, V)
    ws = _ws(nbytes, x)
    y = _empty((N, Cout, T, V), x)
    ok = _launched("agcn_gcn_unit_infer", x, adj, wcat, bias, res, x2, w2, K2, 1 if relu else 0, y, ws, nbytes, N, C, Cout,
                   T, V)
    return y if ok else None


def conv9_infer(x, w, b, res=None, relu=True, stride=1):
    N, Cin, T, V = x.shape
    Cout = w.shape[0]
    To = conv_out_frames(T, 9, stride)
    ws, nbytes = _conv_ws(Cin, Cout, T, V, 9, stride, x)
    y = _empty((N, Cout, To, V), x)
    ok = _launched("agcn_conv9_infer", x, w, b, res, 1 if relu else 0, y, ws, nbytes, N, Cin, Cout, T, V, stride)
    return y if ok else None


def tconv_infer(x, w, b, a_s=None, a_t=None, a_c=None, res=None, relu=True, stride=1, pad=None, x_amax=None):
    N, Cin, T, V = x.shape
    Cout, Cin2, taps, one = w.shape
    assert Cin2 == Cin and one == 1
    pad = (taps - 1) // 2 if pad is None else pad
    To = conv_out_frames(T, taps, stride, pad)
    if To < 1:
        raise ValueError(f"agcn_amd: a {taps}-frame kernel with padding {pad} does not fit {T} frames")
    ws, nbytes = _conv_ws(Cin, Cout, T, V, taps, stride, x, pad)
    y = _empty((N, Cout, To, V), x)
    if not _launched("agcn_tconv_infer", x, w, b, a_s, a_t, a_c, res, 1 if relu else 0, y, ws, nbytes, N, Cin, Cout, T,
                     V, taps, stride, pad, x_amax):
        return None
    INFER_STATS['tconv_infer'] += 1
    return y


def _cache_key(srcs):
    return (_PARAM_EPOCH[0],) + tuple((t.data_ptr(), t._version) for t in srcs if t is not None)


def tcn_infer(x, w, b, bn, stride, pad, cache=None):
    key = _cache_key([w, b, *bn])
    f = cache.get('folded') if cache is not None else None
    if f is None or f[0] != key:
        f = (key,) + _fold_conv(w, b, bn)
        if cache is not None:
            cache['folded'] = f
    return tconv_infer(x.contiguous(), f[1], f[2], relu=False, stride=stride, pad=pad)


_NONE6 = (None,) * 6


def _pack_wb(p):
    wab = bab = None
    if p['ab'] is not None:
        wab = torch.cat([t for wa, _, wb, _ in p['ab'] for t in (wa, wb)], 0)
        bab = torch.cat([t for _, ba, _, bb in p['ab'] for t in (ba, bb)], 0)
    (w0, b0), (w1, b1), (w2, b2) = p['conv_d']
    Cout, C = w0.shape[:2]
    return wab, bab, torch.cat([w0.view(Cout, C), w1.view(Cout, C), w2.view(Cout, C)], dim=1), b0 + b1 + b2


def pack_gcn(p):
    return (p['A'], p['PA'], *_pack_wb(p), *p['gbn'], *(p['down'] or _NONE6))


def pack_tcn(p):
    return (p['tw'], p['tb'], *p['tbn'], p['res_mode'], *(p['res'] or _NONE6), p['stride'])


def _fold_unit(p):
    wab, bab, wd, bd = _pack_wb(p)
    s1, sh1 = _fold(p['gbn'])
    wdf = (wd * s1[:, None]).contiguous()
    bias = bd * s1 + sh1
    w2 = None
    if p['down'] is not None:
        dw, db = p['down'][:2]
        s2, sh2 = _fold(p['down'][2:])
        w2 = (dw.reshape(dw.shape[0], dw.shape[1]) * s2[:, None]).contiguous()
        bias = bias + db * s2 + sh2
    twf, tbf = _fold_conv(p['tw'], p['tb'], p['tbn'])
    rwf, rbf = _fold_conv(*p['res'][:2], p['res'][2:]) if p['res'] is not None else (None, None)
    return wdf, bias.contiguous(), w2, twf, tbf, rwf, rbf, wab, bab


def unit_infer(x, p, cache=None):
    x = x.contiguous()
    N, C, T, V = x.shape
    if C < 32 or _L().agcn_gemm_mode() not in (b'bf16x6', b'bf16'):
        return None
    srcs = [t for wb in p['conv_d'] for t in wb] + [t for q in (p['ab'] or ()) for t in q]
    srcs += [*p['gbn'], p['tw'], p['tb'], *p['tbn'], *(p['down'] or ()), *(p['res'] or ())]
    key = _cache_key(srcs)
    f = cache.get('folded') if cache is not None else None
    if f is None or f[0] != key:
        f = (key,) + _fold_unit(p)
        if cache is not None:
            cache['folded'] = f
    _, wdf, bias, w2, twf, tbf, rwf, rbf, wab, bab = f
    _, adj, _, _ = _adjacency(x, wab, bab, p['A'], p['PA'], p['alpha'], keep_tp=False, x_amax=None, want_amax=False)
    if w2 is None:
        g = gcn_unit_infer(x, adj, wdf, bias, res=x)
    else:
        g = gcn_unit_infer(x, adj, wdf, bias, x2=x, w2=w2)
    if g is None:
        return None
    a_s = a_t = a_c = None
    if p['attn'] is not None:
        _, m_s = stc_row_reduce(g, want_v=True, scale_v=1.0 / T)
        a_s = STCAttentionFunction._gates(m_s, None, *p['attn'])[0]
        mv1, _ = stc_row_reduce(g, wv=a_s, want_t=True, scale_t=1.0 / V)
        _, a_t, a_c, _, _ = STCAttentionFunction._gates(m_s, mv1, *p['attn'], a_s=a_s)
    if p['res_mode'] == 0:
        r = None
    elif p['res_mode'] == 1:
        r = x
    else:
        r, _ = conv_fwd(x, rwf, rbf, p['stride'])
    y = tconv_infer(g, twf, tbf, a_s, a_t, a_c, res=r, relu=True, stride=p['stride'], pad=p['pad'])
    if y is not None:
        INFER_STATS['aagcn_unit_fused'] += 1
    return y


def _axis(pair):
    if pair is None:
        return -1, -1
    j0, j1 = (int(j) for j in pair)
    if j0 < 0 or j1 < 0:
        raise ValueError(f"agcn_amd: joint indices are 0-based and non-negative, got {pair}")
    return j0, j1


def skel_append(ring, frame, slot, count, moving_avg=1):
    Mmax, Tmax, V, C = ring.shape
    if C != 3 or tuple(frame.shape) != (Mmax, V, 3):
        raise ValueError(f"agcn_amd: skel_append takes a ({Mmax}, {V}, 3) frame for this ring, got {tuple(frame.shape)}")
    _lib.call("agcn_skel_append", frame, ring, Mmax, Tmax, V, int(slot), int(count), int(moving_avg))


def prenorm(x, num_select=None, origin=0, frames=None, zaxis=(0, 1), zaxis2=None, xaxis=(8, 4), pad=True, center=True,
            center_firstframe=False):
    if (center or center_firstframe) and center == center_firstframe:
        raise ValueError("agcn_amd: center and center_firstframe exclude each other")
    if x.dim() != 5 or x.shape[-1] != 3:
        raise ValueError(f"agcn_amd: prenorm takes (N, M, T, V, 3), got {tuple(x.shape)}")
    N, M, Tmax, V, _ = x.shape
    T = Tmax if frames is None else int(frames)
    select = num_select is not None
    K = int(num_select) if select else M
    out = _empty((N, 3, T, V, K), x)
    sel = torch.empty((N, K), dtype=torch.int32, device=x.device)
    energy = _empty((N, M), x) if select else None
    (z0, z1), (x0, x1), (zz0, zz1) = _axis(zaxis), _axis(xaxis), _axis(zaxis2)
    _lib.call("agcn_prenorm", x, out, sel, energy, N, M, K, T, Tmax, int(origin), V, 1 if select else 0,
              1 if pad else 0, 1 if center else (2 if center_firstframe else 0), z0, z1, x0, x1, zz0, zz1)
    return out, sel, energy


def _plan(t, n, what):
    if t is not None and (t.dim() != 1 or t.dtype != torch.int32 or (n is not None and t.numel() != n)):
        raise ValueError(f"agcn_amd: {what} must be a 1-D int32 tensor" + (f" of length {n}" if n is not None else "")
                         + f", got {t.dtype} {tuple(t.shape)}")
    return t


def prenorm_windows(pool, start, length, block=None, frames=None, num_select=None, zaxis=(0, 1), zaxis2=None,
                    xaxis=(8, 4), pad=True, center=True, center_firstframe=False):
    if (center or center_firstframe) and center == center_firstframe:
        raise ValueError("agcn_amd: center and center_firstframe exclude each other")
    if pool.dim() != 5 or pool.shape[-1] != 3:
        raise ValueError(f"agcn_amd: prenorm_windows takes a pool (nblocks, M, Tmax, V, 3), got {tuple(pool.shape)}")
    nblocks, M, Tmax, V, _ = pool.shape
    T = Tmax if frames is None else int(frames)
    if not 1 <= T <= Tmax:
        raise ValueError(f"agcn_amd: prenorm_windows needs 1 <= frames <= Tmax = {Tmax}, got {T}")
    if start is None or length is None:
        raise ValueError("agcn_amd: prenorm_windows needs start and length")
    N = _plan(start, None, 'start').numel()
    if N < 1:
        raise ValueError("agcn_amd: prenorm_windows needs at least one window")
    _plan(length, N, 'length')
    _plan(block, N, 'block')
    select = num_select is not None
    K = int(num_select) if select else M
    out = _empty((N, 3, T, V, K), pool)
    sel = torch.empty((N, K), dtype=torch.int32, device=pool.device)
    energy = _empty((N, M), pool) if select else None
    (z0, z1), (x0, x1), (zz0, zz1) = _axis(zaxis), _axis(xaxis), _axis(zaxis2)
    _lib.call("agcn_prenorm_windows", pool, out, sel, energy, block, start, length, N, nblocks, M, K, T, Tmax, V,
              1 if select else 0, 1 if pad else 0, 1 if center else (2 if center_firstframe else 0), z0, z1, x0, x1,
              zz0, zz1)
    return out, sel, energy


def skel_smooth(raw, moving_avg=1):
    if raw.dim() != 4 or raw.shape[-1] != 3:
        raise ValueError(f"agcn_amd: skel_smooth takes a recording (L, Mmax, V, 3), got {tuple(raw.shape)}")
    L, Mmax, V, _ = raw.shape
    if not 1 <= int(moving_avg) <= L:
        raise ValueError(f"agcn_amd: skel_smooth needs 1 <= moving_avg <= L = {L}, got {moving_avg}")
    out = _empty((Mmax, L, V, 3), raw)
    _lib.call("agcn_skel_smooth", raw, out, Mmax, L, V, int(moving_avg))
    return out


def skel_append_many(rings, frames, slot, count, moving_avg=1):
    if rings.dim() != 5 or rings.shape[-1] != 3:
        raise ValueError(f"agcn_amd: skel_append_many takes rings (S, Mmax, Tmax, V, 3), got {tuple(rings.shape)}")
    S, Mmax, Tmax, V, _ = rings.shape
    if tuple(frames.shape) != (S, Mmax, V, 3):
        raise ValueError(f"agcn_amd: skel_append_many takes ({S}, {Mmax}, {V}, 3) frames for these rings, got "
                         f"{tuple(frames.shape)}")
    _plan(slot, S, 'slot')
    _plan(count, S, 'count')
    _lib.call("agcn_skel_append_many", frames, rings, slot, count, S, Mmax, Tmax, V, int(moving_avg))


STREAMS = ('joint', 'bone', 'joint_motion', 'bone_motion')
STREAM_MAX_V = 32


def stream_hip_enabled():
    return os.environ.get('AGCN_STREAM_HIP', '1') != '0'


def _stream_parents(parent, V):
    if torch.is_tensor(parent) or isinstance(parent, np.ndarray):
        parent = parent.tolist()
    parent = tuple(parent)
    if len(parent) != V:
        raise ValueError(f"agcn_amd: the parent table has {len(parent)} entries for {V} joints")
    if any(isinstance(p, bool) or int(p) != p or not 0 <= int(p) < V for p in parent):
        raise ValueError(f"agcn_amd: every parent must be a joint index in [0, {V}), got {list(parent)}")
    return tuple(int(p) for p in parent)

# ... 1453 lines not shown
```

include/agcn_hip.h:

```cpp
#ifndef AGCN_HIP_H
#define AGCN_HIP_H

#include <stddef.h>

#ifdef __cplusplus
extern "C" {
#endif

#define AGCN_OK 0
#define AGCN_ERR_ARG (-1)
#define AGCN_ERR_WORKSPACE (-2)
#define AGCN_ERR_UNSUPPORTED (-3)

int agcn_version(void);
const char* agcn_arch(void);

const char* agcn_last_kernel(void);
const char* agcn_gemm_mode(void);
const char* agcn_chain_mode(void);

int agcn_conv_tile_frames(int V, int T_out);
int agcn_conv_num_tiles(int V, int T_out);
int agcn_conv_stats_tiles(int Cin, int Cout, int T_out, int V, int taps, int stride);
int agcn_scores_num_tiles(int V, int T);
int agcn_dadj_num_slots(int C, int V, int T);

size_t agcn_conv_workspace(int Cin, int Cout, int T, int V, int taps, int stride);
int agcn_conv_fwd(const float* x, const float* w, const float* bias, float* y, float* stats_part, void* workspace,
                  size_t workspace_bytes, int N, int Cin, int Cout, int T, int V, int taps, int stride, void* stream);
int agcn_conv_bwd_data(const float* dy, const float* w, float* dx, int accumulate, const float* add1,
                       const float* mask1, const float* add2, const float* mask2, void* workspace,
                       size_t workspace_bytes, int N, int Cin, int Cout, int T, int V, int taps, int stride,
                       void* stream);
size_t agcn_conv_bwd_weight_workspace(int N, int Cin, int Cout, int T, int V, int taps, int stride);
int agcn_conv_bwd_weight(const float* dy, const float* x, float* dw, void* workspace, size_t workspace_bytes, int N,
                         int Cin, int Cout, int T, int V, int taps, int stride, void* stream);

size_t agcn_gcn_workspace(int C, int Cout, int T, int V);
int agcn_gcn_stats_tiles(int C, int Cout, int T, int V);
int agcn_gcn_stats_slots(int N, int C, int Cout, int T, int V);
int agcn_gcn_aggregate_project_fwd(const float* x, const float* adj, const float* wcat, const float* bias, float* y,
                                   float* stats_part, void* workspace, size_t workspace_bytes, int N, int C, int Cout,
                                   int T, int V, void* stream);
int agcn_bn_act_fwd_ex(const float* y1, const float* scale1, const float* shift1, const float* r, const float* scale2,
                       const float* shift2, float* out, unsigned* sign_bits, float* absmax_out, int N, int C, int P,
                       int res_mode, int relu, void* stream);
int agcn_bn_bwd_apply_ex(const float* part, int nrows, double count, float param_grad_scale, const float* dout,
                         const void* mask, int mask_bits, const float* y1, const float* gamma1, const float* mean1,
                         const float* invstd1, const float* y2, const float* gamma2, const float* mean2,
                         const float* invstd2, float* coef, float* dy1, float* dgamma1, float* dbeta1, float* dy2,
                         float* dgamma2, float* dbeta2, float* absmax1_out, int N, int C, int P, void* stream);
int agcn_gcn_aggregate_project_fwd_ex(const float* x, const float* adj, const float* wcat, const float* bias, float* y,
                                      float* stats_part, void* workspace, size_t workspace_bytes, int N, int C, int Cout,
                                      int T, int V, const float* x_absmax, void* stream);
int agcn_gcn_aggregate_project_bwd_data_ex(const float* dy, const float* adj, const float* wcat, const float* dtp,
                                           const float* w2, int K2, float* dx, int accumulate, const float* add1,
                                           const float* mask1, const float* add2, const float* mask2, int mask_bits,
                                           void* workspace, size_t workspace_bytes, int N, int C, int Cout, int T, int V,
                                           const float* dy_absmax, const float* dtp_absmax, void* stream);
int agcn_gcn_dadj_ex(const float* dy, const float* wcat, const float* x, float* dadj_part, void* workspace,
                     size_t workspace_bytes, int N, int C, int Cout, int T, int V, const float* dy_absmax,
                     const float* x_absmax, void* stream);
int agcn_adjacency_bwd_scores_ex(const float* tp, const float* dS, float* dtp, float* dbpart, void* scratch, float* db,
                                 float* dtp_absmax_out, int N, int Ci, int T, int V, void* stream);
int agcn_conv_bwd_weight_ex(const float* dy, const float* x, float* dw, void* workspace, size_t workspace_bytes, int N,
                            int Cin, int Cout, int T, int V, int taps, int stride, const float* dy_absmax,
                            const float* x_absmax, void* stream);
int agcn_gcn_project_bwd_weight_ex(const float* dy, const float* x, const float* adj, float* dwcat, void* workspace,
                                   size_t workspace_bytes, int N, int C, int Cout, int T, int V, const float* dy_absmax,
                                   const float* x_absmax, void* stream);
int agcn_absmax(const float* x, long n, float* out, void* stream);
int agcn_conv_fwd_ex(const float* x, const float* w, const float* bias, float* y, float* stats_part, void* workspace,
                     size_t workspace_bytes, int N, int Cin, int Cout, int T, int V, int taps, int stride,
                     const float* x_absmax, void* stream);
int agcn_conv_bwd_data_ex(const float* dy, const float* w, float* dx, int accumulate, const float* add1,
                          const float* mask1, const float* add2, const float* mask2, void* workspace,
                          size_t workspace_bytes, int N, int Cin, int Cout, int T, int V, int taps, int stride,
                          const float* dy_absmax, void* stream);

size_t agcn_tconv_workspace(int Cin, int Cout, int T, int V, int taps, int stride, int pad);
int agcn_tconv_stats_tiles(int Cin, int Cout, int T_out, int V, int taps, int stride, int pad);
int agcn_tconv_fwd(const float* x, const float* w, const float* bias, float* y, float* stats_part, void* workspace,
                   size_t workspace_bytes, int N, int Cin, int Cout, int T, int V, int taps, int stride, int pad,
                   const float* x_absmax, void* stream);
int agcn_tconv_bwd_data(const float* dy, const float* w, float* dx, int accumulate, const float* add1,
                        const float* mask1, const float* add2, const float* mask2, void* workspace,
                        size_t workspace_bytes, int N, int Cin, int Cout, int T, int V, int taps, int stride, int pad,
                        const float* dy_absmax, void* stream);
size_t agcn_tconv_bwd_weight_workspace(int N, int Cin, int Cout, int T, int V, int taps, int stride, int pad);
int agcn_tconv_bwd_weight(const float* dy, const float* x, float* dw, void* workspace, size_t workspace_bytes, int N,
                          int Cin, int Cout, int T, int V, int taps, int stride, int pad, const float* dy_absmax,
                          const float* x_absmax, void* stream);

int agcn_gcn_first_supported(int C, int Cout, int V);
int agcn_gcn_first_tiles(int T, int V);
int agcn_gcn_first_fwd(const float* x, const float* adj, const float* wcat, const float* bias, const float* wdown,
                       const float* bdown, float* ypre, float* ystats, float* dpre, float* dstats, int N, int C, int Cout,
                       int T, int V, void* stream);

size_t agcn_gcn_unit_infer_workspace(int C, int Cout, int K2, int T, int V);
int agcn_gcn_unit_infer(const float* x, const float* adj, const float* wcat, const float* bias, const float* res,
                        const float* x2, const float* w2, int K2, int relu, float* y, void* workspace,
                        size_t workspace_bytes, int N, int C, int Cout, int T, int V, void* stream);
int agcn_conv9_infer(const float* x, const float* w, const float* bias, const float* res, int relu, float* y,
                     void* workspace, size_t workspace_bytes, int N, int Cin, int Cout, int T, int V, int stride,
                     void* stream);

int agcn_tconv_infer(const float* x, const float* w, const float* bias, const float* a_s, const float* a_t,
                     const float* a_c, const float* res, int relu, float* y, void* workspace, size_t workspace_bytes,
                     int N, int Cin, int Cout, int T, int V, int taps, int stride, int pad, const float* x_absmax,
                     void* stream);

int agcn_gcn_aggregate_project_bwd_data(const float* dy, const float* adj, const float* wcat, float* dx,
                                        int accumulate, const float* add1, const float* mask1, const float* add2,
                                        const float* mask2, int mask_bits, void* workspace, size_t workspace_bytes, int N, int C,
                                        int Cout, int T, int V, void* stream);
int agcn_gcn_bwd_data_fused_supported(int C, int Cout, int V);
int agcn_gcn_aggregate_project_bwd_data_fused(const float* dy, const float* adj, const float* wcat, const float* dtp,
                                              const float* w2, int K2, float* dx, int accumulate, const float* add1,
                                              const float* mask1, const float* add2, const float* mask2, int mask_bits,
                                              void* workspace, size_t workspace_bytes, int N, int C, int Cout, int T,
                                              int V, void* stream);
size_t agcn_gcn_project_bwd_weight_workspace(int N, int C, int Cout, int T, int V);
int agcn_gcn_project_bwd_weight(const float* dy, const float* x, const float* adj, float* dwcat, void* workspace,
                                size_t workspace_bytes, int N, int C, int Cout, int T, int V, void* stream);
int agcn_gcn_dadj(const float* dy, const float* wcat, const float* x, float* dadj_part, void* workspace,
                  size_t workspace_bytes, int N, int C, int Cout, int T, int V, void* stream);

int agcn_adjacency_fwd(const float* tp, const float* A, const float* PA, const float* alpha, float* spart, float* P,
                       float* adj, int N, int Ci, int T, int V, void* stream);
int agcn_adjacency_fused_supported(int C, int Ci, int T, int V);
size_t agcn_adjacency_fused_workspace(int C, int Ci);
int agcn_adjacency_fused_fwd(const float* x, const float* wab, const float* bab, const float* A, const float* PA,
                             const float* alpha, float* tp_out, float* spart, float* P, float* adj, void* workspace,
                             size_t workspace_bytes, int N, int C, int Ci, int T, int V, void* stream);
int agcn_adjacency_fused_fwd_ex(const float* x, const float* wab, const float* bab, const float* A, const float* PA,
                                const float* alpha, float* tp_out, float* spart, float* P, float* adj, float* x_absmax_out,
                                const float* x_absmax_in, void* workspace, size_t workspace_bytes, int N, int C, int Ci, int T,
                                int V, void* stream);
int agcn_adjacency_fused_bwd_scores(const float* x, const float* wab, const float* bab, const float* dS, float* dtp,
                                    float* dbpart, void* scratch, float* db, void* workspace, size_t workspace_bytes,
                                    int N, int C, int Ci, int T, int V, void* stream);
int agcn_adjacency_bwd_softmax(const float* dadj_part, const float* P, const float* alpha, float* dadj, float* dS,
                               float* dPA, float* dalpha_part, int N, int Ci, int T, int V, int nslots, void* stream);
int agcn_adjacency_bwd_scores(const float* tp, const float* dS, float* dtp, float* dbpart, void* scratch, float* db,
                              int N, int Ci, int T, int V, void* stream);

size_t agcn_colsum_scratch_bytes(int W);
int agcn_colsum(const float* X, int nslots, int W, void* scratch, float* out, void* stream);
int agcn_bn_stats_finalize(const float* stats_part, int nslots, int C, double count, const float* gamma,
                           const float* beta, float* running_mean, float* running_var, float momentum, float eps,
                           void* scratch , float* mean, float* invstd,
                           float* scale, float* shift, void* stream);
int agcn_bn_eval_coeff(const float* gamma, const float* beta, const float* running_mean, const float* running_var,
                       float eps, int C, float* scale, float* shift, void* stream);
int agcn_bn_act_fwd(const float* y1, const float* scale1, const float* shift1, const float* r, const float* scale2,
                    const float* shift2, float* out, unsigned* sign_bits, int N, int C, int P, int res_mode, int relu,
                    void* stream);
int agcn_bn_bwd_reduce(const float* dout, const void* mask, int mask_bits, const float* y1, const float* y2, float* part,
                       int N, int C, int P, void* stream);
int agcn_bn_bwd_apply(const float* part, int nrows, double count, float param_grad_scale, const float* dout,
                      const void* mask, int mask_bits, const float* y1, const float* gamma1, const float* mean1,
                      const float* invstd1, const float* y2, const float* gamma2, const float* mean2, const float* invstd2, float* coef,
                      float* dy1, float* dgamma1, float* dbeta1, float* dy2, float* dgamma2, float* dbeta2, int N, int C,
                      int P, void* stream);
int agcn_bn_bwd(const float* dout, const void* mask, int mask_bits, const float* y1, const float* gamma1,
                const float* mean1, const float* invstd1, const float* y2, const float* gamma2, const float* mean2, const float* invstd2,
                float* part, float* coef, float* dy1, float* dgamma1, float* dbeta1, float* dy2, float* dgamma2,
                float* dbeta2, int N, int C, int P, void* stream);
int agcn_bn_eval_coeff_ex(const float* gamma, const float* beta, const float* running_mean, const float* running_var,
                          float eps, int C, float* scale, float* shift, float* mean, float* invstd, void* stream);
int agcn_bn_bwd_eval(const float* dout, const void* mask, int mask_bits, const float* y1, const float* scale1,
                     const float* y2, const float* scale2, int want_sums, float* part , float* dy1,
                     float* dy2, float* absmax1_out, int N, int C, int P, void* stream);
int agcn_bn_bwd_eval_finalize(const float* part, int nrows, int C, const float* scale1, const float* mean1,
                              const float* invstd1, const float* scale2, const float* mean2, const float* invstd2,
                              float* dgamma1, float* dbeta1, float* dbias1, float* dgamma2, float* dbeta2,
                              float* dbias2, void* stream);

int agcn_stc_row_reduce(const float* y, const float* g, const float* wv, const float* wt, int wt_per_row, float* out_t,
                        float* out_v, float scale_t, float scale_v, int N, int C, int T, int V, void* stream);
int agcn_stc_apply(const float* y, const float* a_s, const float* a_t, const float* a_c, float* out, int N, int C, int T,
                   int V, void* stream);
int agcn_stc_apply_ex(const float* y, const float* a_s, const float* a_t, const float* a_c, float* out, float* absmax_out,
                      int N, int C, int T, int V, void* stream);
int agcn_stc_bwd_apply(const float* dout, const float* a_s, const float* a_t, const float* a_c, const float* dmv,
                       const float* dms, float* dy, int N, int C, int T, int V, void* stream);

int agcn_data_bn_stats(const float* x, float* part, int N, int C, int T, int V, int M, void* stream);
int agcn_data_bn_apply(const float* x, const float* scale, const float* shift, float* out, int N, int C, int T, int V,
                       int M, void* stream);
int agcn_data_bn_bwd_reduce(const float* dy, const float* x, const float* mean, const float* invstd, float* part, int N,
                            int C, int T, int V, int M, void* stream);
int agcn_data_bn_bwd_apply(const float* dy, const float* x, const float* gamma, const float* mean, const float* invstd,
                           const float* sums, double count, float* dx, int N, int C, int T, int V, int M, void* stream);
int agcn_pool_fwd(const float* x, float* rowmean, float* pooled, int N, int M, int C, int P, void* stream);
int agcn_pool_bwd(const float* dpooled, float* dx, int N, int M, int C, int P, void* stream);
int agcn_linear_fwd(const float* in, const float* w, const float* b, float* out, int N, int K, int O, int act,
                    void* stream);
int agcn_linear_bwd(const float* dout, const float* out, const float* in, const float* w, float* dpre, float* din,
                    float* dw, float* db, int N, int K, int O, int act, void* stream);
int agcn_gate_conv_fwd(const float* in, const float* w, const float* b, float* a, int N, int C, int L, int Ks,
                       void* stream);
int agcn_gate_conv_bwd(const float* da, const float* a, const float* in, const float* w, float* dpre, float* din,
                       float* dw, float* db, int N, int C, int L, int Ks, void* stream);

size_t agcn_sgd_step_workspace(long n);
int agcn_sgd_step(float* param, const float* grad, float* momentum_buf, long n, float lr, float momentum,
                  float weight_decay, int nesterov, float max_norm, float grad_scale, int first_step, void* workspace,
                  size_t workspace_bytes, float* norm_out, void* stream);

int agcn_prenorm_max_frames(void);
int agcn_skel_append(const float* frame, float* ring, int Mmax, int Tmax, int V, int slot, int count, int k,
                     void* stream);
int agcn_prenorm(const float* in, float* out, int* sel, float* energy, int N, int M, int K, int T, int Tmax, int origin,
                 int V, int select, int pad, int center, int z0, int z1, int x0, int x1, int zz0, int zz1, void* stream);
int agcn_prenorm_windows(const float* in, float* out, int* sel, float* energy, const int* block, const int* start,
                         const int* len, int N, int nblocks, int M, int K, int T, int Tmax, int V, int select, int pad,
                         int center, int z0, int z1, int x0, int x1, int zz0, int zz1, void* stream);
int agcn_skel_smooth(const float* raw, float* out, int Mmax, int L, int V, int k, void* stream);
int agcn_skel_append_many(const float* frames, float* rings, const int* slot, const int* count, int S, int Mmax,
                          int Tmax, int V, int k, void* stream);

int agcn_tokens_fwd(const float* x, const float* cls, const float* pe, int pe_rows, float* tok, int N, int M, int C,
                    int Tp, int V, void* stream);
int agcn_tokens_bwd(const float* dtok, float* dx, float* dcls, float* dpe, int has_cls, int pe_rows, int N, int M, int C,
                    int Tp, int V, void* stream);
int agcn_mha_fwd(const float* qkv, const unsigned char* null_tok, int causal, const unsigned char* keep, float keep_scale,
                 float* ctx, float* prob, float* avg, int N, int L, int H, int dh, void* stream);
int agcn_mha_bwd(const float* dctx, const float* qkv, const float* prob, const unsigned char* keep, float keep_scale,
                 float* dqkv, void* ws, size_t ws_bytes, int N, int L, int H, int dh, void* stream);
int agcn_ln_fwd(const float* a, const float* b, const float* gamma, const float* beta, float eps, float* out, float* mean,
                float* rstd, long R, int D, void* stream);
int agcn_ln_bwd(const float* dy, const float* a, const float* b, const float* gamma, const float* mean, const float* rstd,
                float* dx, float* dgamma, float* dbeta, void* ws, size_t ws_bytes, long R, int D, void* stream);

int agcn_tokens_spatial_fwd(const float* x, const float* cls, const float* pe, int pe_rows, float* tok, int N, int M,
                            int C, int Tp, int V, void* stream);
size_t agcn_tokens_spatial_bwd_workspace(int N, int M, int C, int Tp, int V, int has_cls);
int agcn_tokens_spatial_bwd(const float* dtok, float* dx, float* dcls, float* dpe, int has_cls, int pe_rows, void* ws,
                            size_t ws_bytes, int N, int M, int C, int Tp, int V, void* stream);
int agcn_mha_bias_fwd(const float* qkv, const float* bias, int Hb, const unsigned char* null_tok, int causal,
                      const unsigned char* keep, float keep_scale, float* ctx, float* prob, float* avg, int N, int L,
                      int H, int dh, void* stream);
size_t agcn_mha_bias_grad_workspace(int N, int L, int H, int Hb);
int agcn_mha_bias_grad(const float* ds, float* dbias, void* ws, size_t ws_bytes, int N, int L, int H, int Hb,
                       void* stream);

size_t agcn_sgn_frames_weights(int V);
size_t agcn_sgn_clip_weights(int seg, int num_class);
int agcn_sgn_frames(const float* x, const float* w, size_t w_floats, float* feat, float* g, int N, int seg, int V,
                    void* stream);
int agcn_sgn_clip(const float* feat, const float* w, size_t w_floats, float* logits, int N, int seg, int num_class,
                  void* stream);
int agcn_sgn_sample(const float* win, const unsigned* r, float* out, int* L, int N, int T, int V, int K, int S, int seg,
                    void* stream);

int agcn_sgn_collate(const float* pool, const long long* index, const unsigned* r, const float* angles, float* out,
                     float* subj, int* L, long P, int N, int T, int V, int K, int S, int seg, void* stream);

size_t agcn_sgn_frames_bwd_weights(int V);
size_t agcn_sgn_clip_bwd_weights(int seg, int num_class);
size_t agcn_sgn_frames_bwd_workspace(int N, int seg, int V);
int agcn_sgn_clip_bwd(const float* feat, const float* w, size_t w_floats, const float* wt, size_t wt_floats,
                      const float* dlogits, float* dfeat, int N, int seg, int num_class, void* stream);
int agcn_sgn_frames_bwd(const float* x, const float* w, size_t w_floats, const float* wt, size_t wt_floats,
                        const float* dfeat, float* dx, void* ws, size_t ws_bytes, int N, int seg, int V, void* stream);
int agcn_sgn_sample_bwd(const float* win, const unsigned* r, const float* dout, float* dwin, int N, int T, int V, int K,
                        int S, int seg, void* stream);

size_t agcn_sgn_frames_tape_floats(int N, int seg, int V);
size_t agcn_sgn_clip_tape_floats(int N, int seg, int num_class);
size_t agcn_sgn_wgrad_workspace(int N, int seg, int V, int num_class, int rows_per_split);
int agcn_sgn_clip_bwd_tape(const float* feat, const float* w, size_t w_floats, const float* wt, size_t wt_floats,
                           const float* dlogits, float* dfeat, int N, int seg, int num_class, float* tape,
                           size_t tape_floats, void* stream);
int agcn_sgn_frames_bwd_tape(const float* x, const float* w, size_t w_floats, const float* wt, size_t wt_floats,
                             const float* dfeat, float* dx, void* ws, size_t ws_bytes, int N, int seg, int V, float* tape,
                             size_t tape_floats, void* stream);
int agcn_sgn_frames_wgrad(const float* x, const float* w, const float* tape, float* d_w, void* ws, size_t ws_bytes, int N,
                          int seg, int V, int rows_per_split, void* stream);
int agcn_sgn_clip_wgrad(const float* tape, const float* dfeat, const float* dlogits, float* d_w, void* ws, size_t ws_bytes,
                        int N, int seg, int num_class, int rows_per_split, void* stream);

size_t agcn_sgn_stats_part_floats(int kind, int layer, int N, int seg, int V);
size_t agcn_sgn_stats_channels(int kind, int layer, int V);
int agcn_sgn_input_stats(const float* x, float* part, size_t part_floats, int N, int seg, int V, void* stream);
int agcn_sgn_frames_stats(const float* x, const float* w, size_t w_floats, float* part, size_t part_floats, int layer,
                          int N, int seg, int V, void* stream);
int agcn_sgn_clip_stats(const float* feat, const float* w, size_t w_floats, float* part, size_t part_floats, int layer,
                        int N, int seg, int num_class, void* stream);
size_t agcn_sgn_stats_finalize_workspace(int kind, int layer, int N, int seg, int V);
int agcn_sgn_stats_finalize(const float* part, size_t part_floats, int kind, int layer, int N, int seg, int V,
                            const double* carry_in, double* carry_out, float* mean, float* var, void* ws, size_t ws_bytes,
                            void* stream);

size_t agcn_sgn15_frames_weights(int V, int heads, int d_head, int ff);
size_t agcn_sgn15_clip_weights(int seg, int num_class, int heads, int d_head, int ff);
int agcn_sgn15_frames(const float* x, const float* w, size_t w_floats, float* feat, float* attn, int N, int seg, int V,
                      int heads, int d_head, int ff, void* stream);
int agcn_sgn15_clip(const float* feat, const float* w, size_t w_floats, float* logits, float* attn, int N, int seg,
                    int num_class, int heads, int d_head, int ff, void* stream);

size_t agcn_sgn15_frames_bwd_weights(int V, int heads, int d_head, int ff);
size_t agcn_sgn15_clip_bwd_weights(int seg, int num_class, int heads, int d_head, int ff);
size_t agcn_sgn15_frames_bwd_workspace(int N, int seg, int V);
int agcn_sgn15_clip_bwd(const float* feat, const float* w, size_t w_floats, const float* wt, size_t wt_floats,
                        const float* dlogits, float* dfeat, int N, int seg, int num_class, int heads, int d_head, int ff,
                        void* stream);
int agcn_sgn15_frames_bwd(const float* x, const float* w, size_t w_floats, const float* wt, size_t wt_floats,
                          const float* dfeat, float* dx, void* ws, size_t ws_bytes, int N, int seg, int V, int heads,
                          int d_head, int ff, void* stream);

size_t agcn_sgn15_frames_tape_floats(int N, int seg, int V, int heads, int d_head, int ff);
size_t agcn_sgn15_clip_tape_floats(int N, int seg, int num_class, int heads, int d_head, int ff);
size_t agcn_sgn15_wgrad_workspace(int N, int seg, int V, int num_class, int heads, int d_head, int ff, int rows_per_split);
int agcn_sgn15_clip_bwd_tape(const float* feat, const float* w, size_t w_floats, const float* wt, size_t wt_floats,
                             const float* dlogits, float* dfeat, int N, int seg, int num_class, int heads, int d_head,
                             int ff, float* tape, size_t tape_floats, void* stream);
int agcn_sgn15_frames_bwd_tape(const float* x, const float* w, size_t w_floats, const float* wt, size_t wt_floats,
                               const float* dfeat, float* dx, void* ws, size_t ws_bytes, int N, int seg, int V, int heads,
                               int d_head, int ff, float* tape, size_t tape_floats, void* stream);
int agcn_sgn15_frames_wgrad(const float* x, const float* tape, size_t tape_floats, float* d_w, size_t d_w_floats, void* ws,
                            size_t ws_bytes, int N, int seg, int V, int heads, int d_head, int ff, int rows_per_split,
                            void* stream);
int agcn_sgn15_clip_wgrad(const float* tape, size_t tape_floats, const float* dlogits, float* d_w, size_t d_w_floats,
                          void* ws, size_t ws_bytes, int N, int seg, int num_class, int heads, int d_head, int ff,
                          int rows_per_split, void* stream);

size_t agcn_sgn15_stats_part_floats(int kind, int layer, int N, int seg, int V);
size_t agcn_sgn15_stats_channels(int kind, int layer);
int agcn_sgn15_frames_stats(const float* x, const float* w, size_t w_floats, float* part, size_t part_floats, int layer,
                            int N, int seg, int V, int heads, int d_head, int ff, void* stream);
int agcn_sgn15_clip_stats(const float* feat, const float* w, size_t w_floats, float* part, size_t part_floats, int layer,
                          int N, int seg, int num_class, int heads, int d_head, int ff, void* stream);
size_t agcn_sgn15_stats_finalize_workspace(int kind, int layer, int N, int seg, int V);
int agcn_sgn15_stats_finalize(const float* part, size_t part_floats, int kind, int layer, int N, int seg, int V,
                              const double* carry_in, double* carry_out, float* mean, float* var, void* ws, size_t ws_bytes,
                              void* stream);

int agcn_streams_fwd(const float* x, float* bone, float* joint_motion, float* bone_motion, const int* host_parent, int N,
                     int C, int T, int V, int M, void* stream);
int agcn_streams_bwd(const float* d_joint, const float* d_bone, const float* d_joint_motion, const float* d_bone_motion,
                     float* dx, const int* host_parent, float w_joint, float w_bone, float w_joint_motion,
                     float w_bone_motion, int N, int C, int T, int V, int M, void* stream);

#ifdef __cplusplus
}
#endif
#endif
```

Baseline: 1021 clips/s.

## Fold BN stat finalize and bwd coefficient reduce into last-block-done kernels

Batch-norm statistics finalize is merged into the column-sum kernel: each block publishes its partials and draws an atomic ticket, and the last block computes mean, invstd, scale and shift. It also bumps the tick counter and zeroes the amax words, which removes a separate memset. The backward reduce does the same per channel with padded counters, so the last row for each channel folds the partial sums into the coefficients. The aim is to remove several small kernel launches and host-side ops per BN layer, at the cost of atomic counter state that must be reset correctly and serialised tail work in a single block.

```diff
diff --git a/2s-agcn_amd/csrc/bn.hip b/2s-agcn_amd/csrc/bn.hip
--- a/2s-agcn_amd/csrc/bn.hip
+++ b/2s-agcn_amd/csrc/bn.hip
@@ -3,10 +3,10 @@
 namespace {
 
 constexpr int RG = 64;
-
-__global__ void __launch_bounds__(256)
-colsum_stage1_kernel(const float* __restrict__ X, int nslots, int W, int per_group, double* __restrict__ partial) {
-  __shared__ double red[4][64];
+constexpr int BWD_COUNTER_STRIDE = 32;
+
+__device__ __forceinline__ double colsum_stage1_sum(const float* __restrict__ X, int nslots, int W, int per_group,
+                                                    double (*red)[64]) {
   const int col = blockIdx.x * 64 + (threadIdx.x & 63), sub = threadIdx.x >> 6;
   const int g = blockIdx.y;
   const int s_end = min(nslots, (g + 1) * per_group);
@@ -15,8 +15,43 @@
     for (int s = g * per_group + sub; s < s_end; s += 4) acc += (double)X[(long)s * W + col];
   red[sub][threadIdx.x & 63] = acc;
   __syncthreads();
-  if (sub == 0 && col < W)
-    partial[(long)g * W + col] = red[0][threadIdx.x] + red[1][threadIdx.x] + red[2][threadIdx.x] + red[3][threadIdx.x];
+  const int l = threadIdx.x & 63;
+  return red[0][l] + red[1][l] + red[2][l] + red[3][l];
+}
+
+__global__ void __launch_bounds__(256)
+colsum_stage1_kernel(const float* __restrict__ X, int nslots, int W, int per_group, double* __restrict__ partial) {
+  __shared__ double red[4][64];
+  const int col = blockIdx.x * 64 + (threadIdx.x & 63), sub = threadIdx.x >> 6;
+  const double v = colsum_stage1_sum(X, nslots, W, per_group, red);
+  if (sub == 0 && col < W) partial[(long)blockIdx.y * W + col] = v;
+}
+
+__device__ __forceinline__ void publish_f32(float* p, float v) {
+  __hip_atomic_store(reinterpret_cast<unsigned*>(p), __float_as_uint(v), __ATOMIC_RELAXED, __HIP_MEMORY_SCOPE_AGENT);
+}
+__device__ __forceinline__ void publish_f64(double* p, double v) {
+  __hip_atomic_store(reinterpret_cast<unsigned long long*>(p), (unsigned long long)__double_as_longlong(v),
+                     __ATOMIC_RELAXED, __HIP_MEMORY_SCOPE_AGENT);
+}
+__device__ __forceinline__ float collect_f32(const float* p) {
+  return __uint_as_float(__hip_atomic_load(reinterpret_cast<const unsigned*>(p), __ATOMIC_RELAXED,
+                                           __HIP_MEMORY_SCOPE_AGENT));
+}
+__device__ __forceinline__ double collect_f64(const double* p) {
+  return __longlong_as_double((long long)__hip_atomic_load(reinterpret_cast<const unsigned long long*>(p),
+                                                           __ATOMIC_RELAXED, __HIP_MEMORY_SCOPE_AGENT));
+}
+__device__ __forceinline__ unsigned draw_ticket(unsigned* counter) {
+  asm volatile("s_waitcnt vmcnt(0)" ::: "memory");
+  return __hip_atomic_fetch_add(counter, 1u, __ATOMIC_RELAXED, __HIP_MEMORY_SCOPE_AGENT);
+}
+__device__ __forceinline__ void acquire_partials() {
+  __builtin_amdgcn_fence(__ATOMIC_ACQUIRE, "agent");
+  asm volatile("s_waitcnt vmcnt(0)" ::: "memory");
+}
+__device__ __forceinline__ void reset_counter(unsigned* counter) {
+  __hip_atomic_store(counter, 0u, __ATOMIC_RELAXED, __HIP_MEMORY_SCOPE_AGENT);
 }
 
 __global__ void colsum_stage2_kernel(const double* __restrict__ partial, int W, float* __restrict__ out) {
@@ -27,18 +62,12 @@
   out[col] = (float)s;
 }
 
-__global__ void bn_stats_finalize_kernel(const double* __restrict__ partial, int C, double count,
-                                         const float* __restrict__ gamma, const float* __restrict__ beta,
-                                         float* __restrict__ rmean, float* __restrict__ rvar, float momentum,
-                                         float eps, float* __restrict__ mean_out, float* __restrict__ invstd_out,
-                                         float* __restrict__ scale_out, float* __restrict__ shift_out) {
-  const int c = blockIdx.x * blockDim.x + threadIdx.x;
-  if (c >= C) return;
-  double s = 0.0, ss = 0.0;
-  for (int g = 0; g < RG; ++g) {
-    s += partial[((long)g * 2 + 0) * C + c];
-    ss += partial[((long)g * 2 + 1) * C + c];
-  }
+__device__ __forceinline__ void bn_stats_channel(int c, double s, double ss, double count,
+                                                 const float* __restrict__ gamma, const float* __restrict__ beta,
+                                                 float* __restrict__ rmean, float* __restrict__ rvar, float momentum,
+                                                 float eps, float* __restrict__ mean_out,
+                                                 float* __restrict__ invstd_out, float* __restrict__ scale_out,
+                                                 float* __restrict__ shift_out) {
   const double mean = s / count;
   double var = ss / count - mean * mean;
   if (var < 0.0) var = 0.0;
@@ -52,6 +81,61 @@
     const double unb = count > 1.0 ? var * count / (count - 1.0) : var;
     rmean[c] = (1.f - momentum) * rmean[c] + momentum * (float)mean;
     rvar[c] = (1.f - momentum) * rvar[c] + momentum * (float)unb;
+  }
+}
+
+__global__ void bn_stats_finalize_kernel(const double* __restrict__ partial, int C, double count,
+                                         const float* __restrict__ gamma, const float* __restrict__ beta,
+                                         float* __restrict__ rmean, float* __restrict__ rvar, float momentum,
+                                         float eps, float* __restrict__ mean_out, float* __restrict__ invstd_out,
+                                         float* __restrict__ scale_out, float* __restrict__ shift_out) {
+  const int c = blockIdx.x * blockDim.x + threadIdx.x;
+  if (c >= C) return;
+  double s = 0.0, ss = 0.0;
+  for (int g = 0; g < RG; ++g) {
+    s += partial[((long)g * 2 + 0) * C + c];
+    ss += partial[((long)g * 2 + 1) * C + c];
+  }
+  bn_stats_channel(c, s, ss, count, gamma, beta, rmean, rvar, momentum, eps, mean_out, invstd_out, scale_out,
+                   shift_out);
+}
+
+__global__ void __launch_bounds__(256)
+bn_stats_fold_kernel(const float* __restrict__ X, int nslots, int C, int per_group, double* __restrict__ partial,
+                     unsigned* __restrict__ counter, double count, const float* __restrict__ gamma,
+                     const float* __restrict__ beta, float* __restrict__ rmean, float* __restrict__ rvar,
+                     float momentum, float eps, float* __restrict__ mean_out, float* __restrict__ invstd_out,
+                     float* __restrict__ scale_out, float* __restrict__ shift_out, long long* __restrict__ tick,
+                     unsigned* __restrict__ zero0, unsigned* __restrict__ zero1) {
+  __shared__ double red[4][64];
+  __shared__ int last;
+  const int W = 2 * C;
+  const int col = blockIdx.x * 64 + (threadIdx.x & 63), sub = threadIdx.x >> 6;
+  const double v = colsum_stage1_sum(X, nslots, W, per_group, red);
+  if (sub == 0) {
+    if (col < W) publish_f64(partial + (long)blockIdx.y * W + col, v);
+    if (threadIdx.x == 0) {
+      const unsigned total = gridDim.x * gridDim.y;
+      last = draw_ticket(counter) == total - 1u;
+    }
+  }
+  __syncthreads();
+  if (!last) return;
+  acquire_partials();
+  for (int c = threadIdx.x; c < C; c += 256) {
+    double s = 0.0, ss = 0.0;
+    for (int g = 0; g < RG; ++g) {
+      s += collect_f64(partial + ((long)g * 2 + 0) * C + c);
+      ss += collect_f64(partial + ((long)g * 2 + 1) * C + c);
+    }
+    bn_stats_channel(c, s, ss, count, gamma, beta, rmean, rvar, momentum, eps, mean_out, invstd_out, scale_out,
+                     shift_out);
+  }
+  if (threadIdx.x == 0) {
+    reset_counter(counter);
+    if (tick) *tick += 1;
+    if (zero0) *zero0 = 0u;
+    if (zero1) *zero1 = 0u;
   }
 }
 
@@ -123,11 +207,9 @@
 }
 
 template <bool HAS2>
-__global__ void __launch_bounds__(256)
-bn_bwd_reduce_kernel(const float* __restrict__ dout, const float* __restrict__ mask, int mask_bits,
-                     const float* __restrict__ y1, const float* __restrict__ y2, float* __restrict__ part, int P) {
-  __shared__ float red[3][4];
-  const long row = blockIdx.x;
+__device__ __forceinline__ void bn_bwd_row_sums(const float* __restrict__ dout, const float* __restrict__ mask,
+                                                int mask_bits, const float* __restrict__ y1,
+                                                const float* __restrict__ y2, int P, long row, float (*red)[4]) {
   const float* d = dout + row * P;
   const float* mk = (mask && !mask_bits) ? mask + row * P : nullptr;
   const unsigned* mb = (mask && mask_bits) ? reinterpret_cast<const unsigned*>(mask) : nullptr;
@@ -184,9 +266,47 @@
   const int wave = threadIdx.x >> 6;
   if ((threadIdx.x & 63) == 0) { red[0][wave] = s0; red[1][wave] = s1; red[2][wave] = s2; }
   __syncthreads();
+}
+
+template <bool HAS2>
+__global__ void __launch_bounds__(256)
+bn_bwd_reduce_kernel(const float* __restrict__ dout, const float* __restrict__ mask, int mask_bits,
+                     const float* __restrict__ y1, const float* __restrict__ y2, float* __restrict__ part, int P) {
+  __shared__ float red[3][4];
+  const long row = blockIdx.x;
+  bn_bwd_row_sums<HAS2>(dout, mask, mask_bits, y1, y2, P, row, red);
   if (threadIdx.x < 3) {
     const int k = threadIdx.x;
     part[row * 3 + k] = red[k][0] + red[k][1] + red[k][2] + red[k][3];
+  }
+}
+
+__device__ __forceinline__ void bn_bwd_channel(int c, int C, double s0, double s1, double s2, double count, float pscale,
+                                               const float* __restrict__ gamma1, const float* __restrict__ mean1,
+                                               const float* __restrict__ invstd1, const float* __restrict__ gamma2,
+                                               const float* __restrict__ mean2, const float* __restrict__ invstd2,
+                                               float* __restrict__ coef, float* __restrict__ dgamma1,
+                                               float* __restrict__ dbeta1, float* __restrict__ dgamma2,
+                                               float* __restrict__ dbeta2) {
+  {
+    const double is = invstd1[c], mu = mean1[c], g = gamma1[c];
+    const double sxh = is * (s1 - mu * s0);
+    const double k = g * is;
+    coef[0 * C + c] = (float)k;
+    coef[1 * C + c] = (float)(-k * is * sxh / count);
+    coef[2 * C + c] = (float)(-k * s0 / count + k * is * mu * sxh / count);
+    dgamma1[c] = (float)sxh * pscale;
+    dbeta1[c] = (float)s0 * pscale;
+  }
+  if (gamma2) {
+    const double is = invstd2[c], mu = mean2[c], g = gamma2[c];
+    const double sxh = is * (s2 - mu * s0);
+    const double k = g * is;
+    coef[3 * C + c] = (float)k;
+    coef[4 * C + c] = (float)(-k * is * sxh / count);
+    coef[5 * C + c] = (float)(-k * s0 / count + k * is * mu * sxh / count);
+    dgamma2[c] = (float)sxh * pscale;
+    dbeta2[c] = (float)s0 * pscale;
   }
 }
 
@@ -205,25 +325,52 @@
     const float* p = part + ((long)n * C + c) * 3;
     s0 += (double)p[0]; s1 += (double)p[1]; s2 += (double)p[2];
   }
-  {
-    const double is = invstd1[c], mu = mean1[c], g = gamma1[c];
-    const double sxh = is * (s1 - mu * s0);
-    const double k = g * is;
-    coef[0 * C + c] = (float)k;
-    coef[1 * C + c] = (float)(-k * is * sxh / count);
-    coef[2 * C + c] = (float)(-k * s0 / count + k * is * mu * sxh / count);
-    dgamma1[c] = (float)sxh * pscale;
-    dbeta1[c] = (float)s0 * pscale;
-  }
-  if (gamma2) {
-    const double is = invstd2[c], mu = mean2[c], g = gamma2[c];
-    const double sxh = is * (s2 - mu * s0);
-    const double k = g * is;
-    coef[3 * C + c] = (float)k;
-    coef[4 * C + c] = (float)(-k * is * sxh / count);
-    coef[5 * C + c] = (float)(-k * s0 / count + k * is * mu * sxh / count);
-    dgamma2[c] = (float)sxh * pscale;
-    dbeta2[c] = (float)s0 * pscale;
+  bn_bwd_channel(c, C, s0, s1, s2, count, pscale, gamma1, mean1, invstd1, gamma2, mean2, invstd2, coef, dgamma1, dbeta1,
+                 dgamma2, dbeta2);
+}
+
+template <bool HAS2>
+__global__ void __launch_bounds__(256)
+bn_bwd_reduce_fold_kernel(const float* __restrict__ dout, const float* __restrict__ mask, int mask_bits,
+                          const float* __restrict__ y1, const float* __restrict__ y2, float* __restrict__ part, int P,
+                          int N, int C, double count, float pscale, const float* __restrict__ gamma1,
+                          const float* __restrict__ mean1, const float* __restrict__ invstd1,
+                          const float* __restrict__ gamma2, const float* __restrict__ mean2,
+                          const float* __restrict__ invstd2, float* __restrict__ coef, float* __restrict__ dgamma1,
+                          float* __restrict__ dbeta1, float* __restrict__ dgamma2, float* __restrict__ dbeta2,
+                          unsigned* __restrict__ zero_word, unsigned* __restrict__ counters) {
+  __shared__ float red[3][4];
+  const long row = blockIdx.x;
+  bn_bwd_row_sums<HAS2>(dout, mask, mask_bits, y1, y2, P, row, red);
+  if (threadIdx.x >= 64) return;
+  const int c = (int)(row % C);
+  unsigned ticket = 0;
+  if (threadIdx.x == 0) {
+    if (row == 0 && zero_word) *zero_word = 0u;
+#pragma unroll
+    for (int k = 0; k < 3; ++k) publish_f32(part + row * 3 + k, red[k][0] + red[k][1] + red[k][2] + red[k][3]);
+    ticket = draw_ticket(counters + (long)c * BWD_COUNTER_STRIDE);
+  }
+  ticket = (unsigned)__shfl((int)ticket, 0);
+  if (ticket != (unsigned)N - 1u) return;
+  acquire_partials();
+  double s0 = 0.0, s1 = 0.0, s2 = 0.0;
+  for (int n0 = 0; n0 < N; n0 += 64) {
+    const int n = n0 + (int)threadIdx.x;
+    float v0 = 0.f, v1 = 0.f, v2 = 0.f;
+    if (n < N) {
+      const float* p = part + ((long)n * C + c) * 3;
+      v0 = collect_f32(p); v1 = collect_f32(p + 1); v2 = collect_f32(p + 2);
+    }
+    const int m = min(64, N - n0);
+    for (int j = 0; j < m; ++j) {
+      s0 += (double)__shfl(v0, j); s1 += (double)__shfl(v1, j); s2 += (double)__shfl(v2, j);
+    }
+  }
+  if (threadIdx.x == 0) {
+    bn_bwd_channel(c, C, s0, s1, s2, count, pscale, gamma1, mean1, invstd1, gamma2, mean2, invstd2, coef, dgamma1,
+                   dbeta1, dgamma2, dbeta2);
+    reset_counter(counters + (long)c * BWD_COUNTER_STRIDE);
   }
 }
 
@@ -326,6 +473,23 @@
   return agcn_check_launch();
 }
 
+size_t agcn_bn_counter_bytes(int C) { return sizeof(unsigned) * (size_t)BWD_COUNTER_STRIDE * (size_t)(C > 0 ? C : 1); }
+
+int agcn_bn_stats_fold(const float* part, int nslots, int C, double count, const float* gamma, const float* beta,
+                       float* running_mean, float* running_var, float momentum, float eps, void* scratch,
+                       unsigned* counters, float* mean, float* invstd, float* scale, float* shift, long long* tick_word,
+                       float* zero_word0, float* zero_word1, void* stream) {
+  if (!part || !gamma || !beta || !scratch || !counters || !mean || !invstd || !scale || !shift || C <= 0 ||
+      nslots <= 0)
+    return AGCN_ERR_ARG;
+  const int W = 2 * C;
+  const int per_group = (nslots + RG - 1) / RG;
+  hipLaunchKernelGGL(bn_stats_fold_kernel, dim3((W + 63) / 64, RG), dim3(256), 0, (hipStream_t)stream, part, nslots, C,
+                     per_group, (double*)scratch, counters, count, gamma, beta, running_mean, running_var, momentum,
+                     eps, mean, invstd, scale, shift, tick_word, (unsigned*)zero_word0, (unsigned*)zero_word1);
+  return agcn_check_launch();
+}
+
 int agcn_bn_eval_coeff(const float* gamma, const float* beta, const float* running_mean, const float* running_var,
                        float eps, int C, float* scale, float* shift, void* stream) {
   if (!gamma || !beta || !running_mean || !running_var || !scale || !shift || C <= 0) return AGCN_ERR_ARG;
@@ -345,6 +509,14 @@
                        int res_mode, int relu, void* stream) {
   if (!y1 || !scale1 || !shift1 || !out || N <= 0 || C <= 0 || P <= 0) return AGCN_ERR_ARG;
   if (absmax_out && hipMemsetAsync(absmax_out, 0, 4, (hipStream_t)stream) != hipSuccess) return AGCN_ERR_ARG;
+  return agcn_bn_act_fwd_prezeroed(y1, scale1, shift1, r, scale2, shift2, out, sign_bits, absmax_out, N, C, P, res_mode,
+                                   relu, stream);
+}
+
+int agcn_bn_act_fwd_prezeroed(const float* y1, const float* scale1, const float* shift1, const float* r,
+                              const float* scale2, const float* shift2, float* out, unsigned* sign_bits,
+                              float* absmax_out, int N, int C, int P, int res_mode, int relu, void* stream) {
+  if (!y1 || !scale1 || !shift1 || !out || N <= 0 || C <= 0 || P <= 0) return AGCN_ERR_ARG;
   const long total = (long)N * C * P;
   if (total % 4 != 0 || total > 0xffffffffL) return AGCN_ERR_UNSUPPORTED;
   if (res_mode != 0 && !r) return AGCN_ERR_ARG;
@@ -402,6 +574,38 @@
                      dbeta1, dgamma2, dbeta2);
   int rc = agcn_check_launch();
   if (rc) return rc;
+  return agcn_bn_bwd_apply_coef(coef, dout, mask, mask_bits, y1, y2, dy1, dy2, absmax1_out, N, C, P, stream);
+}
+
+int agcn_bn_bwd_reduce_coef(const float* dout, const void* mask, int mask_bits, const float* y1, const float* y2,
+                            float* part, double count, float param_grad_scale, const float* gamma1, const float* mean1,
+                            const float* invstd1, const float* gamma2, const float* mean2, const float* invstd2,
+                            float* coef, float* dgamma1, float* dbeta1, float* dgamma2, float* dbeta2,
+                            float* absmax1_out, unsigned* counters, int N, int C, int P, void* stream) {
+  if (!dout || !y1 || !part || !counters || !gamma1 || !mean1 || !invstd1 || !coef || !dgamma1 || !dbeta1 || N <= 0 ||
+      C <= 0 || P <= 0)
+    return AGCN_ERR_ARG;
+  if (y2 && (!gamma2 || !mean2 || !invstd2 || !dgamma2 || !dbeta2)) return AGCN_ERR_ARG;
+  const long total = (long)N * C * P;
+  if (total % 4 != 0 || total > 0xffffffffL) return AGCN_ERR_UNSUPPORTED;
+  hipStream_t s = (hipStream_t)stream;
+#define LAUNCH_REDUCE_FOLD(H)                                                                                       \
+  hipLaunchKernelGGL(bn_bwd_reduce_fold_kernel<H>, dim3(N * C), dim3(256), 0, s, dout, (const float*)mask, mask_bits, \
+                     y1, y2, part, P, N, C, count, param_grad_scale, gamma1, mean1, invstd1,                        \
+                     y2 ? gamma2 : nullptr, mean2, invstd2, coef, dgamma1, dbeta1, dgamma2, dbeta2,                 \
+                     (unsigned*)absmax1_out, counters)
+  if (y2) LAUNCH_REDUCE_FOLD(true); else LAUNCH_REDUCE_FOLD(false);
+#undef LAUNCH_REDUCE_FOLD
+  return agcn_check_launch();
+}
+
+int agcn_bn_bwd_apply_coef(const float* coef, const float* dout, const void* mask, int mask_bits, const float* y1,
+                           const float* y2, float* dy1, float* dy2, float* absmax1_out, int N, int C, int P,
+                           void* stream) {
+  if (!coef || !dout || !y1 || !dy1 || (y2 && !dy2) || N <= 0 || C <= 0 || P <= 0) return AGCN_ERR_ARG;
+  const long total = (long)N * C * P;
+  if (total % 4 != 0 || total > 0xffffffffL) return AGCN_ERR_UNSUPPORTED;
+  hipStream_t s = (hipStream_t)stream;
   const unsigned t4 = (unsigned)(total / 4);
   const dim3 g(ew_grid(t4)), b(256);
   if (y2)
diff --git a/2s-agcn_amd/lib.py b/2s-agcn_amd/lib.py
--- a/2s-agcn_amd/lib.py
+++ b/2s-agcn_amd/lib.py
@@ -15,7 +15,8 @@
 _BITS32, _ANY = ("int32", (torch.int32, torch.uint32)), ("", None)
 _POINTERS = {"float*": _FP32, "const float*": _FP32, "double*": _FP64, "const double*": _FP64,
              "int*": _INT32, "const int*": _INT32, "unsigned*": _BITS32, "const unsigned*": _BITS32,
-             "const long long*": ("int64", (torch.int64,)), "const unsigned char*": ("uint8", (torch.uint8,)),
+             "const long long*": ("int64", (torch.int64,)), "long long*": ("int64", (torch.int64,)),
+             "const unsigned char*": ("uint8", (torch.uint8,)),
              "void*": _ANY, "const void*": _ANY}
 _TYPE_WORDS = {"const", "void", "char", "int", "long", "unsigned", "signed", "short", "float", "double", "size_t"}
 
diff --git a/2s-agcn_amd/model/agcn.py b/2s-agcn_amd/model/agcn.py
--- a/2s-agcn_amd/model/agcn.py
+++ b/2s-agcn_amd/model/agcn.py
@@ -67,10 +67,9 @@
 def data_bn_forward(bn, x):
     N, C, T, V, M = x.size()
     if ops.data_bn_supported(bn):
-        y = ops.DataBNFunction.apply(x, bn.weight, bn.bias, bn.running_mean, bn.running_var, bn.training,
-                                     ops.sync_of(bn))
-        _bn_tick(bn, bn.training)
-        return y
+        with ops.bn_ticks(bn.training, bn):
+            return ops.DataBNFunction.apply(x, bn.weight, bn.bias, bn.running_mean, bn.running_var, bn.training,
+                                            ops.sync_of(bn))
     x = x.permute(0, 4, 3, 1, 2).contiguous().view(N, M * V * C, T)
     x = bn(x)
     return x.view(N, M, V, C, T).permute(0, 1, 3, 4, 2).contiguous().view(N * M, C, T, V)
@@ -93,10 +92,9 @@
 
     def forward(self, x):
         _require_gpu(x, 'unit_tcn')
-        y = ops.UnitTCNFunction.apply(x, self.conv.weight, self.conv.bias, *_bn_args(self.bn), self.stride,
-                                      self.training, ops.sync_of(self.bn), self.pad)
-        _bn_tick(self.bn, self.training)
-        return y
+        with ops.bn_ticks(self.training, self.bn):
+            return ops.UnitTCNFunction.apply(x, self.conv.weight, self.conv.bias, *_bn_args(self.bn), self.stride,
+                                             self.training, ops.sync_of(self.bn), self.pad)
 
 
 class unit_gcn(nn.Module):
@@ -137,16 +135,14 @@
     def params(self):
         return gcn_params(self, self, self.A, self.PA)
 
-    def tick(self):
-        _bn_tick(self.bn, self.training)
-        if isinstance(self.down, nn.Sequential):
-            _bn_tick(self.down[1], self.training)
+    def bns(self):
+        return [self.bn] + ([self.down[1]] if isinstance(self.down, nn.Sequential) else [])
 
     def forward(self, x):
         _require_gpu(x, 'unit_gcn')
-        y = ops.UnitGCNFunction.apply(x, *ops.pack_gcn(self.params()), self.training, None, ops.sync_of(self.bn))
-        self.tick()
-        return y
+        with ops.bn_ticks(self.training, *self.bns()):
+            return ops.UnitGCNFunction.apply(x, *ops.pack_gcn(self.params()), self.training, None,
+                                             ops.sync_of(self.bn))
 
 
 class TCN_GCN_unit(nn.Module):
@@ -178,12 +174,10 @@
             y = ops.unit_infer(x, p, cache=self.__dict__.setdefault('_infer_cache', {}))
             if y is not None:
                 return y
-        y = ops.TCNGCNUnitFunction.apply(x, *ops.pack_gcn(p), *ops.pack_tcn(p), self.training, ops.sync_of(t.bn))
-        self.gcn1.tick()
-        _bn_tick(t.bn, self.training)
-        if self.res_mode == 2:
-            _bn_tick(self.residual.bn, self.training)
-        return y
+        bns = self.gcn1.bns() + [t.bn] + ([self.residual.bn] if self.res_mode == 2 else [])
+        with ops.bn_ticks(self.training, *bns):
+            return ops.TCNGCNUnitFunction.apply(x, *ops.pack_gcn(p), *ops.pack_tcn(p), self.training,
+                                                ops.sync_of(t.bn))
 
 
 class Model(nn.Module):
diff --git a/2s-agcn_amd/ops.py b/2s-agcn_amd/ops.py
--- a/2s-agcn_amd/ops.py
+++ b/2s-agcn_amd/ops.py
@@ -455,11 +455,12 @@
 
 
 class BNState:
-    __slots__ = ("mean", "invstd", "scale", "shift", "S", "eval")
+    __slots__ = ("mean", "invstd", "scale", "shift", "S", "eval", "zeroed")
 
     def __init__(self):
         self.S = 1
         self.eval = False
+        self.zeroed = None
 
 
 class SyncBN:
@@ -507,15 +508,58 @@
     return out
 
 
-def bn_train_coeffs(stats_part, count, gamma, beta, running_mean, running_var, momentum=BN_MOMENTUM, eps=BN_EPS):
+_COUNTERS = {}
+
+
+def _counters(C, like):
+    stream = torch.cuda.current_stream(like.device)
+    key = (stream.device_index, stream.cuda_stream)
+    words = _L().agcn_bn_counter_bytes(int(C)) // 4
+    buf = _COUNTERS.get(key)
+    if buf is None or buf.numel() < words:
+        with torch.cuda.stream(stream):
+            buf = _COUNTERS[key] = torch.zeros(max(words, 8192), dtype=torch.int32, device=like.device)
+    return buf
+
+
+_TICKS = {}
+
+
+class bn_ticks:
+
+    def __init__(self, training, *bns):
+        bns = [bn for bn in bns if training and bn.num_batches_tracked is not None]
+        self.words = {bn.running_mean.data_ptr(): bn.num_batches_tracked for bn in bns
+                      if bn.num_batches_tracked.is_cuda}
+        self.rest = [bn for bn in bns if not bn.num_batches_tracked.is_cuda]
+
+    def __enter__(self):
+        _TICKS.update(self.words)
+        return self
+
+    def __exit__(self, exc_type, exc, tb):
+        for key, word in self.words.items():
+            if _TICKS.pop(key, None) is not None and exc_type is None:
+                word.add_(1)
+        if exc_type is None:
+            for bn in self.rest:
+                bn.num_batches_tracked.add_(1)
+        return False
+
+
+def bn_train_coeffs(stats_part, count, gamma, beta, running_mean, running_var, momentum=BN_MOMENTUM, eps=BN_EPS,
+                    zero=None):
     C = gamma.numel()
     st = BNState()
     st.mean, st.invstd = _empty((C,), gamma), _empty((C,), gamma)
     st.scale, st.shift = _empty((C,), gamma), _empty((C,), gamma)
     nslots = stats_part.shape[0]
     scratch = _scratch(2 * C, gamma)
-    _lib.call("agcn_bn_stats_finalize", stats_part, nslots, C, float(count), gamma, beta, running_mean, running_var,
-              float(momentum), float(eps), scratch, st.mean, st.invstd, st.scale, st.shift)
+    tick = _TICKS.pop(running_mean.data_ptr(), None) if running_mean is not None else None
+    _lib.call("agcn_bn_stats_fold", stats_part, nslots, C, float(count), gamma, beta, running_mean, running_var,
+              float(momentum), float(eps), scratch, _counters(C, gamma), st.mean, st.invstd, st.scale, st.shift, tick,
+              zero, None)
+    st.zeroed = zero
     return st
 
 
@@ -537,7 +581,8 @@
     out = torch.empty_like(y1)
     bits = torch.empty((y1.numel() + 31) // 32, dtype=torch.int32, device=y1.device) if want_bits else None
     mode = 0 if r is None else (1 if st2 is None else 2)
-    _lib.call("agcn_bn_act_fwd_ex", y1, st1.scale, st1.shift, r, st2.scale if st2 else None, st2.shift if st2 else None,
+    entry = "agcn_bn_act_fwd_prezeroed" if amax_out is not None and st1.zeroed is amax_out else "agcn_bn_act_fwd_ex"
+    _lib.call(entry, y1, st1.scale, st1.shift, r, st2.scale if st2 else None, st2.shift if st2 else None,
               out, bits, amax_out, N, C, T * V, mode, int(relu))
     return (out, bits) if want_bits else out
 
@@ -574,6 +619,13 @@
 
 def _bn_bwd_two_stage(grad, ins, outs, part, coef, amax_out, N, C, TV, sync, gcount):
     dout, mptr, mbits = grad
+    if sync is None:
+        y1, g1, m1, i1, y2, g2, m2, i2 = ins
+        dy1, dg1, db1, dy2, dg2, db2 = outs
+        _lib.call("agcn_bn_bwd_reduce_coef", dout, mptr, mbits, y1, y2, part, float(N) * float(TV), 1.0, g1, m1, i1,
+                  g2, m2, i2, coef, dg1, db1, dg2, db2, amax_out, _counters(C, dout), N, C, TV)
+        _lib.call("agcn_bn_bwd_apply_coef", coef, dout, mptr, mbits, y1, y2, dy1, dy2, amax_out, N, C, TV)
+        return
     _lib.call("agcn_bn_bwd_reduce", dout, mptr, mbits, ins[0], ins[4], part, N, C, TV)
     sums, nslots, total, scale = part, N, float(N) * float(TV), 1.0
     if sync is not None:
@@ -643,7 +695,7 @@
         self.wres, self.gamma2, self.stride, self.relu, self.pad = wres, gamma2, stride, relu, pad
 
 
-def _bn_coeffs(training, stats, count, bns, sync=None, nsamples=None):
+def _bn_coeffs(training, stats, count, bns, sync=None, nsamples=None, zero=None):
     S = bns[0][2].numel() // bns[0][0].numel()
     if not training:
         out = []
@@ -661,7 +713,8 @@
         stats = sync_stats(stats, count, sync)
         count = count * sync.world
     note_params_changed()
-    res = [bn_train_coeffs(sp, count, *bn) for sp, bn in zip(stats, bns)]
+    res = [bn_train_coeffs(sp, count, *bn, zero=zero if i == 0 else None)
+           for i, (sp, bn) in enumerate(zip(stats, bns))]
     for st in res:
         st.S = S
     return res, count
@@ -701,13 +754,13 @@
     else:
         ypre, st = aggregate_project_fwd(x, adj, wd, bd, want_stats=training, x_amax=x_amax)
         dpre, st2 = conv_fwd(x, down[0], down[1], want_stats=training) if down is not None else (None, None)
+    g_amax = _empty((1,), x) if fused_amax_enabled() else None
     if down is not None:
-        (bn1, bn2), gcount = _bn_coeffs(training, [st, st2], count, [bn, down[2:]], sync, N)
+        (bn1, bn2), gcount = _bn_coeffs(training, [st, st2], count, [bn, down[2:]], sync, N, zero=g_amax)
         r = dpre
     else:
-        (bn1,), gcount = _bn_coeffs(training, [st], count, [bn], sync, N)
+        (bn1,), gcount = _bn_coeffs(training, [st], count, [bn], sync, N, zero=g_amax)
         bn2, r = None, x
-    g_amax = _empty((1,), x) if fused_amax_enabled() else None
     out, bits = bn_act_fwd(ypre, bn1, r, bn2, relu=True, want_bits=True, amax_out=g_amax)
     wdown, gamma2 = (down[0], down[2]) if down is not None else (None, None)
     return out, _GCNState(x, tp, P, adj, ypre, dpre, bits, bn1, bn2, sync, gcount, x_amax, g_amax, wab, bab, wd, bn[0],
@@ -769,14 +822,14 @@
     To = zpre.shape[2]
     count = N * To * V
     rpre = bn2 = wres = gamma2 = None
+    o_amax = _empty((1,), g) if fused_amax_enabled() else None
     if res is None or isinstance(res, str):
-        (bn1,), gcount = _bn_coeffs(training, [st], count, [bn], sync, N)
+        (bn1,), gcount = _bn_coeffs(training, [st], count, [bn], sync, N, zero=o_amax)
         r = None if res is None else res_x
     else:
         r, st2 = conv_fwd(res_x, res[0], res[1], stride, want_stats=training)
-        (bn1, bn2), gcount = _bn_coeffs(training, [st, st2], count, [bn, res[2:]], sync, N)
+        (bn1, bn2), gcount = _bn_coeffs(training, [st, st2], count, [bn, res[2:]], sync, N, zero=o_amax)
         rpre, wres, gamma2 = r, res[0], res[2]
-    o_amax = _empty((1,), g) if fused_amax_enabled() else None
     out, bits = bn_act_fwd(zpre, bn1, r, bn2, relu=relu, want_bits=True, amax_out=o_amax)
     _note_out_amax(out, o_amax)
     return out, _TCNState(g, zpre, rpre, out, bits, bn1, bn2, sync, gcount, g_amax, res_x, w, bn[0], wres, gamma2,
diff --git a/include/agcn_hip.h b/include/agcn_hip.h
--- a/include/agcn_hip.h
+++ b/include/agcn_hip.h
@@ -152,6 +152,12 @@
                            const float* beta, float* running_mean, float* running_var, float momentum, float eps,
                            void* scratch , float* mean, float* invstd,
                            float* scale, float* shift, void* stream);
+size_t agcn_bn_counter_bytes(int C);
+int agcn_bn_stats_fold(const float* stats_part, int nslots, int C, double count, const float* gamma, const float* beta,
+                       float* running_mean, float* running_var, float momentum, float eps,
+                       void* scratch , unsigned* counters, float* mean,
+                       float* invstd, float* scale, float* shift, long long* tick_word, float* zero_word0,
+                       float* zero_word1, void* stream);
 int agcn_bn_eval_coeff(const float* gamma, const float* beta, const float* running_mean, const float* running_var,
                        float eps, int C, float* scale, float* shift, void* stream);
 int agcn_bn_act_fwd(const float* y1, const float* scale1, const float* shift1, const float* r, const float* scale2,
@@ -168,6 +174,17 @@
                 const float* mean1, const float* invstd1, const float* y2, const float* gamma2, const float* mean2, const float* invstd2,
                 float* part, float* coef, float* dy1, float* dgamma1, float* dbeta1, float* dy2, float* dgamma2,
                 float* dbeta2, int N, int C, int P, void* stream);
+int agcn_bn_bwd_reduce_coef(const float* dout, const void* mask, int mask_bits, const float* y1, const float* y2,
+                            float* part, double count, float param_grad_scale, const float* gamma1, const float* mean1,
+                            const float* invstd1, const float* gamma2, const float* mean2, const float* invstd2,
+                            float* coef, float* dgamma1, float* dbeta1, float* dgamma2, float* dbeta2,
+                            float* absmax1_out, unsigned* counters, int N, int C, int P, void* stream);
+int agcn_bn_bwd_apply_coef(const float* coef, const float* dout, const void* mask, int mask_bits, const float* y1,
+                           const float* y2, float* dy1, float* dy2, float* absmax1_out, int N, int C, int P,
+                           void* stream);
+int agcn_bn_act_fwd_prezeroed(const float* y1, const float* scale1, const float* shift1, const float* r,
+                              const float* scale2, const float* shift2, float* out, unsigned* sign_bits,
+                              float* absmax_out, int N, int C, int P, int res_mode, int relu, void* stream);
 int agcn_bn_eval_coeff_ex(const float* gamma, const float* beta, const float* running_mean, const float* running_var,
                           float eps, int C, float* scale, float* shift, float* mean, float* invstd, void* stream);
 int agcn_bn_bwd_eval(const float* dout, const void* mask, int mask_bits, const float* y1, const float* scale1,
```

After: 1020 clips/s. About the same (-0.2%).
